# iyak/RNAelem

Hardware: AMD Instinct MI355X
Metric: train-iter seqs/sec (inside+outside) (higher is better)
Workload: dtype f64; 1 GPU; 10000 synthetic RNAs L=200, pattern ((.*.)), W=50 C=30 min_bpp=1e-4 T2004, x0 lambda=(1,1), one (fn,gr) eval per step; n_seq=10000, seq_len=200, pattern=((.*.)), bpp_filter=cached (computed once at load_batch, 0.1 s incl. plan), n_skipped=0

## Files before the change

### rnaelem_amd/api.py

```python
import ctypes as C
import json
import os

import numpy as np

HERE = os.path.dirname(os.path.abspath(__file__))
LIB_PATH = os.path.join(HERE, "libelemdp.so")

NO_RSS, NO_PROFILE, NO_ENERGY, THETA_SOFTMAX, LIK_RATIO = 1, 2, 4, 8, 16
DBG_FIX_RSS, DBG_NO_TURN = 1 << 9, 1 << 10

SYMBOLS = ["elemdp_last_error", "elemdp_abi_version", "elemdp_set_data_dir", "elemdp_create", "elemdp_destroy",
           "elemdp_n_param", "elemdp_n_state", "elemdp_n_node", "elemdp_initial_params", "elemdp_describe",
           "elemdp_set_option", "elemdp_load_batch", "elemdp_batch_bpp_eff", "elemdp_batch_pairs", "elemdp_useful_mask", "elemdp_useful_mask_host", "elemdp_live_blocks", "elemdp_live_blocks_host", "elemdp_live_blocks_inside", "elemdp_live_blocks_host_bits", "elemdp_train_eval",
           "elemdp_partial_len", "elemdp_train_partial", "elemdp_train_finish", "elemdp_set_finish_params", "elemdp_train_seq_stats", "elemdp_train_seq_counts",
           "elemdp_debug_tables", "elemdp_scan", "elemdp_pair_posteriors", "elemdp_pair_mea", "elemdp_sample", "elemdp_context_profile", "elemdp_node_profile", "elemdp_accessibility", "elemdp_node_mea", "elemdp_pair_conditional", "elemdp_pair_conditional_list", "elemdp_pair_list", "elemdp_last_timing", "elemdp_debug_profile", "elemdp_kernel_name", "elemdp_kmer_shuffle", "elemdp_epoch_permutation",
           "elemdp_comm_unique_id", "elemdp_comm_init", "elemdp_comm_destroy"]


class ModelDesc(C.Structure):
    _fields_ = [("pattern", C.c_char_p), ("energy_param", C.c_char_p), ("max_span", C.c_int32), ("max_iloop", C.c_int32),
                ("min_bpp", C.c_double), ("tau", C.c_double), ("flags", C.c_int32), ("device", C.c_int32)]


# ... 384 lines not shown
                r["structure_motif"] = sm.raw[lo:hi].decode("ascii")
                r["structure_none"] = sn.raw[lo:hi].decode("ascii")
            recs.append(r)
        return recs

    SAMPLED, NO_PARSE, REFUSED = 0, 1, 2

    def sample_structures(self, x, n_samples, seed=0, index_base=0):
        x = np.ascontiguousarray(x, dtype=np.float64)
        off = self._off
        n_samples = int(n_samples)
        nb = max(int(off[-1]) * max(n_samples, 0), 1)
        rss = C.create_string_buffer(nb)
        node = np.zeros(nb, dtype=np.uint8)
        logp = np.zeros(max(self.n_seq * max(n_samples, 0), 1))
        status = np.zeros(max(self.n_seq, 1), dtype=np.int32)
        self._check(self._lib.elemdp_sample(self._h, _dp(x), self.n_param, n_samples, int(seed) & (2 ** 64 - 1), int(index_base),
                                            rss, node.ctypes.data_as(C.POINTER(C.c_uint8)), _dp(logp), _i32(status)))
        raw = rss.raw.decode("ascii")
        out = []
        for k in range(self.n_seq):
            L, b = int(off[k + 1] - off[k]), int(off[k]) * n_samples
            out.append(([raw[b + t * L:b + (t + 1) * L] for t in range(n_samples)], node[b:b + n_samples * L].reshape(n_samples, L).copy(),
                        logp[k * n_samples:(k + 1) * n_samples].copy(), int(status[k])))
        return out

    CONTEXT_LETTERS = "OLRHBIM"

    def context_profiles(self, x):
        x = np.ascontiguousarray(x, dtype=np.float64)
        off = self._off
        n_pos = int(off[-1]) if off is not None else 0
        prof = np.zeros(max(7 * n_pos, 1))
        self._check(self._lib.elemdp_context_profile(self._h, _dp(x), self.n_param, _dp(prof)))
        return [prof[7 * int(off[k]):7 * int(off[k + 1])].reshape(-1, 7).copy() for k in range(self.n_seq)]

    def node_profiles(self, x):
        x = np.ascontiguousarray(x, dtype=np.float64)
        off = self._off
        M = self.n_node
        n_pos = int(off[-1]) if off is not None else 0
        prof = np.zeros(max(M * n_pos, 1))
        self._check(self._lib.elemdp_node_profile(self._h, _dp(x), self.n_param, _dp(prof)))
        return [prof[M * int(off[k]):M * int(off[k + 1])].reshape(-1, M).copy() for k in range(self.n_seq)]

    def accessibility(self, x, max_width=16):
        x = np.ascontiguousarray(x, dtype=np.float64)
        off = self._off
        U = int(max_width)
        n_pos = int(off[-1]) if off is not None else 0
        acc = np.zeros(max(max(U, 1) * n_pos, 1))
        self._check(self._lib.elemdp_accessibility(self._h, _dp(x), self.n_param, U, _dp(acc)))
        return [acc[U * int(off[k]):U * int(off[k + 1])].reshape(-1, U).copy() for k in range(self.n_seq)]

    def mea_alignments(self, x, gamma=1.0, max_sites=1, profile=False):
        x = np.ascontiguousarray(x, dtype=np.float64)
        off = self._off
        M, K, n = self.n_node, int(max_sites), max(self.n_seq, 0)
        n_pos = int(off[-1]) if off is not None else 0
        kk = min(max(K, 1), 64)
        prof = np.zeros(max(M * n_pos, 1)) if profile else None
        node = np.zeros(max(kk * n_pos, 1), dtype=np.uint8)
        ns = np.zeros(max(n, 1), dtype=np.int32)
        s0, s1 = np.zeros(max(n * kk, 1), dtype=np.int32), np.zeros(max(n * kk, 1), dtype=np.int32)
        sc, cf = np.zeros(max(n * kk, 1)), np.zeros(max(n * kk, 1))
        self._check(self._lib.elemdp_node_mea(self._h, _dp(x), self.n_param, float(gamma), K, _dp(prof), _u8(node), _i32(ns),
                                              _i32(s0), _i32(s1), _dp(sc), _dp(cf)))
        out = []
        for k in range(self.n_seq):
            a, b, m = int(off[k]), int(off[k + 1]), int(ns[k])
            L = b - a
            rec = dict(rows=node[K * a:K * a + m * L].reshape(m, L).copy(), start=s0[k * K:k * K + m].copy(),
                       end=s1[k * K:k * K + m].copy(), score=sc[k * K:k * K + m].copy(), confidence=cf[k * K:k * K + m].copy())
            if profile:
                rec["profile"] = prof[M * a:M * b].reshape(L, M).copy()
            out.append(rec)
        return out

    def last_timing(self):
        ms = np.zeros(3)
        self._lib.elemdp_last_timing(self._h, _dp(ms), 3)
        return ms

    def profile(self):
        c = np.zeros(16)
        self._lib.elemdp_debug_profile(self._h, _dp(c), 16)
        return c

    def kernel_name(self):
        return self._lib.elemdp_kernel_name().decode()


def alignment_confidence(profile, psihat):
    profile = np.asarray(profile, dtype=np.float64)
    psihat = np.asarray(psihat, dtype=np.int64)
    if profile.ndim != 2 or psihat.shape != (profile.shape[0],):
        raise ValueError("alignment_confidence: an (L, M) profile and L node indices are expected")
    if psihat.size and (psihat.min() < 0 or psihat.max() >= profile.shape[1]):
        raise ValueError("alignment_confidence: node index out of range")
    return profile[np.arange(profile.shape[0]), psihat]
```

### rnaelem_amd/csrc/engine.cpp

```cpp
#include <hip/hip_runtime_api.h>

#include <algorithm>
#include <chrono>
#include <cmath>
#include <cstdio>
#include <cstdlib>
#include <cstring>
#include <fstream>
#include <limits>
#include <memory>
#include <numeric>
#include <random>
#include <sstream>
#include <stdexcept>
#include <string>
#include <mutex>
#include <thread>
#include <vector>

#include <dlfcn.h>

#include "../../include/elemdp.h"
#include "access_rules.h"
#include "automaton.h"
// ... 105 lines not shown
  DevBuf d_plans, dmin, e_stack, e_ext, e_ml, e_close, e_hp, off_outer, off_inner, off_left, off_right, cursor, items,
      item_in, idx_inner, idx_left, idx_right, items_inner, items_left, items_right;
  DevBuf useful;
  bool useful_built = false;
  DevBuf blocks, blk_max;
  int64_t n_blocks = 0;
  int blk_cpb = 0, blk_cap = 0;
  std::vector<int32_t> h_blk_max, h_blk_grid;
  std::vector<int32_t> h_blk_grid_in;
  bool blk_all = false;
  bool blk_two = false;
  int64_t n_cells = 0;
  bool permuted = false;
  bool inner_only = false;
  bool sorted = true;
  PlanKernelArgs ka;
  int64_t n_items = 0;
  PlanArrays arrays() const {
    PlanArrays a;
    a.dmin = dmin.as<int16_t>();
    a.e_stack = e_stack.as<double>(); a.e_ext = e_ext.as<double>(); a.e_ml = e_ml.as<double>();
    a.e_close = e_close.as<double>(); a.e_hp = e_hp.as<double>();
    a.by_outer_off = off_outer.as<int32_t>(); a.by_inner_off = off_inner.as<int32_t>();
    a.by_left_off = off_left.as<int32_t>(); a.by_right_off = off_right.as<int32_t>();
    a.cursor = cursor.as<int32_t>();
    a.items = items.as<LoopItem>(); a.item_in = item_in.as<uint8_t>();
    a.by_inner_idx = idx_inner.as<int32_t>(); a.by_left_idx = idx_left.as<int32_t>(); a.by_right_idx = idx_right.as<int32_t>();
    a.items_inner = items_inner.as<LoopItem>(); a.items_left = items_left.as<LoopItem>(); a.items_right = items_right.as<LoopItem>();
    return a;
  }
};

}

class Engine {
 public:
  explicit Engine(const elemdp_model_desc& d);
  ~Engine();

  void useful_mask(int idx, uint8_t* mask, int cap);
  void live_blocks(int idx, int32_t* counts, void* records, int stride, int32_t* cpb_cap, int32_t* taken, bool inside = false);
  int n_param() const { return au_.n_theta() + 2; }
  int n_state() const { return au_.S(); }
  int n_node() const { return au_.M(); }
  const Automaton& automaton() const { return au_; }
  const AutomatonLayout& layout() const { return lays_.shadow >= 0 ? lays_ : lay_; }
  bool softmax() const { return flags_ & ELEMDP_THETA_SOFTMAX; }

  void load_batch(const uint8_t* seq, const int32_t* off, const uint8_t* qual, const int32_t* qoff, const char* fix, int n);
  void train_partial(const double* x, int n_param, void* partial, bool device_ptr, bool reduce = false);
  void train_finish(const double* reduced, double* fn, double* gr, double* sum_eff, int32_t* n_skipped);
  void scan(const double* x, int n_param, elemdp_scan_out* out);
  struct MeaOut { double gamma; char* structure; double* score; };
  void pair_posteriors(const double* x, int n_param, double min_prob, int64_t* n_pairs, double* unpaired, const MeaOut* mea = nullptr);
  void pair_list(int32_t* seq, int32_t* i, int32_t* j, double* p, int64_t cap);
  struct CondOut { double gamma; double* exist; double* unpaired[2]; char* structure[2]; double* shift; };
  void pair_conditional(const double* x, int n_param, double min_prob, int64_t* n_pairs, const CondOut& out);
  void cond_list(int32_t* seq, int32_t* i, int32_t* j, double* p_motif, double* p_none, int64_t cap);
  struct SampleOut { char* rss; uint8_t* node; double* logp; int32_t* status; };
  void sample_structures(const double* x, int n_param, int n_samples, uint64_t seed, int64_t index_base, const SampleOut& out);
  void context_profile(const double* x, int n_param, double* profile);
  void node_profile(const double* x, int n_param, double* profile);
  void accessibility(const double* x, int n_param, int max_width, double* access);
  struct NodeMeaOut { double* profile; uint8_t* node; int32_t* n_sites; int32_t* start; int32_t* end; double* score; double* conf; };
  void node_mea(const double* x, int n_param, double gamma, int max_sites, const NodeMeaOut& out);
  int partial_len() const { return 4 + 2 * au_.n_theta() + 4; }
  void set_option(const std::string& key, double v);
  void comm_init(int rank, int world, const void* id);
  void comm_destroy();
  bool has_comm() const { return comm_ != nullptr; }

  int n_seq() const { return n_seq_; }
  const std::vector<SeqPlan>& plans() const { return h_plans_; }
  void seq_stats(double* out, int n);
  void seq_counts(double* out, int n);
  bool bpp_eff_known() const {
    if (!streaming_) return true;
    for (char c : st_have_eff_) if (!c) return false;
    return true;
  }
  void debug_tables(double* inside, double* outside, double* inside_o, double* outside_o, double* ENo, double* ENx, double* EH);
  void batch_pairs(int idx, uint8_t* kept, double* lnbpp, int cap);
  double last_ms[3] = {0, 0, 0};

 private:
  void upload_params(const double* x, const AutomatonLayout& lay, bool trivial);
 public:
  void set_theta_from(const double* x);
 private:
  struct BatchShape {
    std::vector<SeqPlan> plans;
    int Lmax = 0, Wmax = 0, nword_max = 0;
    int64_t n_bases = 0, n_pos = 0, n_words = 0, n_cells = 0;
  };
  BatchShape check_batch(const uint8_t* seq, const int32_t* off, const uint8_t* qual, const int32_t* qoff, const char* fix, int n) const;
  void stage_batch(BatchShape&& b, const uint8_t* seq, const int32_t* off, const uint8_t* qual, const int32_t* qoff, const char* fix,
                   std::vector<uint8_t>& h_seq, std::vector<uint32_t>& fix_bits);
  const uint32_t* bpp_filter(const std::vector<uint32_t>& fix_bits);
  void bpp_chunks(bool lin);
  void bpp_lin_chunk(int first, int count, int64_t cells, double* lnbpp);
  void bpp_log_chunk(int first, int count, int64_t cells, double* lnbpp);
  void resident_plan(const uint32_t* mask);
  void build_planset(PlanSet& ps, int first, int count, const uint32_t* d_okbits);
  void ensure_sorted_plan();
  void ensure_useful_mask();
  bool ensure_live_blocks(int cpb, int cap, bool inside_too);
  bool loop_prepass_ok(bool sched1) const;
  bool loop_outside_ok(bool sched1) const;
  int live_span_for(int cpb) const;
  bool lists_wanted() const;
  LdsLayout lds_layout(const AutomatonLayout& lay, int Lmax, int nword_max, bool scan) const;
  DpArgs base_args(const AutomatonLayout& lay, const int32_t* d_ints, const double* d_params, const PlanSet& ps,
                   const uint32_t* d_okbits, int S);
  SlotRequest slot_request(int S, int row, bool scan, int n_want, int group = 0, int pair_row = 0) const;
  void run_train();
  void run_train_batch();
  void run_lin_batch();
  int prepare_lin(LinArgs& a, bool sched1, bool dense_too = false, int n_eval = 0, int group_cap = 8192);
  template <class Work> void sweep_groups(const LinArgs& a, int n, const int32_t* h_ord, const int32_t* d_ord, const SeqPlan* d_sorted,
                                          int gsz, int ns, Work work);
  struct ScanPos {
    DevBuf start, inner, end, ys, ye, exist;
    ScanPos(size_t n_seqpos, int n) {
      start.alloc(8 * n_seqpos); inner.alloc(8 * n_seqpos); end.alloc(8 * (n_seqpos + n));
      ys.alloc(4 * (size_t)n); ye.alloc(4 * (size_t)n); exist.alloc(8 * (size_t)n);
    }
  };
  int prepare_scan(LinArgs& a, const ScanPos& pos);
  int read_flagged(std::vector<int32_t>* list = nullptr);
  DpArgs log_scan_args(bool sums_on_batch, int* n_blocks);
  int log_chunk(bool sums_on_batch, int n_blocks, int n_log) const;
  PairArgs pair_batch_args() const;
  void pair_plane_fields(PairArgs& pa, const LinArgs& a) const;
  void require_resident(const char* what, int n_param_in);
  template <class Fill, class Group> int scan_sums(const ScanPos& pos, Fill fill, Group group, std::vector<int32_t>* flagged = nullptr);
  template <class Fill, class Behind> void scan_log_form(bool sums_on_batch, int n_flagged, Fill fill, Behind behind);
  int node_profile_device(const char* what, const double* x, int n_param_in);
  TrArgs log_pipeline_args();
  void init_device();
  void flatten_automaton();
  void poison_tables();
  void lin_weights(int first = 0, int count = 0);
  void upload_automaton();
  bool opt_prune_ = true;
  int opt_eval_first_ = 0, opt_eval_count_ = 0;
  std::vector<int32_t> h_order_r_;
  DevBuf d_order_r_, d_plans_sorted_r_;
  int range_key_[2] = {-1, -1};
  bool opt_det_ = false;
  bool opt_fast_ = true;
  bool opt_poison_ = false;
  void require_device() const;
  bool has_device_ = false;
  int want_device_ = -1;
  Rccl::Comm comm_ = nullptr;
  int comm_rank_ = 0, comm_world_ = 1;
  bool streaming_ = false;
  int st_chunk_ = 0, opt_max_resident_ = 0;
  bool inner_ = false;
  size_t slot_budget_ = 0, st_slot_budget_ = 0;
  std::vector<uint8_t> st_seq_, st_qual_;
  std::vector<char> st_fix_;
  std::vector<double> st_rows_;
  std::unique_ptr<Engine> sub_[2];
  std::vector<std::pair<std::string, double>> opt_log_;
  elemdp_model_desc desc_;
  std::string desc_pattern_, desc_par_;
  bool desc_has_par_ = false;
  bool should_stream(const BatchShape& b);
  void stream_setup(const uint8_t* seq, const int32_t* off, const uint8_t* qual, const int32_t* qoff, const char* fix,
                    BatchShape&& b);
  void stream_load_chunk(int k, Engine& e);
  std::vector<std::vector<uint32_t>> st_mask_;
  std::vector<std::vector<double>> st_eff_;
  std::vector<char> st_have_eff_;
  const uint32_t* preset_bits_ = nullptr;
  const double* preset_eff_ = nullptr;
  size_t preset_words_ = 0;
  size_t bits_words_ = 0;
  void set_filter_preset(const uint32_t* bits, size_t words, const double* eff) { preset_bits_ = bits; preset_words_ = words; preset_eff_ = eff; }
  void filter_result(std::vector<uint32_t>& bits, std::vector<double>& eff) {
    bits.resize(bits_words_);
    HIP_OK(hipMemcpyAsync(bits.data(), d_okbits1_.as<void>(), sizeof(uint32_t) * bits_words_, hipMemcpyDeviceToHost, st_));
    HIP_OK(hipStreamSynchronize(st_));
    eff.resize(h_plans_.size());
    for (size_t k = 0; k < h_plans_.size(); ++k) eff[k] = h_plans_[k].bpp_eff;
  }
  void stream_subs();
  template <class Checked, class Work> void stream_call(int n_param_in, Checked checked, Work work);
  void stream_train(const double* x, int n_param, void* partial, bool device_ptr, bool reduce);
  void stream_scan(const double* x, int n_param, elemdp_scan_out* out);
  void stream_pairs(const double* x, int n_param, double min_prob, double* unpaired, const MeaOut* mea);
  void stream_samples(const double* x, int n_param, int n_samples, uint64_t seed, int64_t index_base, const SampleOut& out);
  void stream_cond(const double* x, int n_param, double min_prob, const CondOut& out);
  DevBuf d_pr_kept_, d_pr_koff_, d_pr_cnt_, d_pr_off_, d_pr_P_, d_pr_unp_, d_pr_si_, d_pr_sj_, d_pr_sp_;
  DevBuf d_pl_seq_, d_pl_i_, d_pl_j_, d_pl_p_;
  int64_t n_pairs_ = -1;
  DevBuf d_mea_M_, d_mea_ch_, d_mea_s_, d_mea_sc_;
  DevBuf d_sm_rss_, d_sm_node_, d_sm_logp_, d_sm_status_, d_sm_stack_;
  DevBuf d_cd_kept_, d_cd_koff_, d_cd_cnt_, d_cd_off_, d_cd_P_, d_cd_z_, d_cd_unp_[2], d_cd_exist_, d_cd_shift_, d_cd_si_, d_cd_sj_, d_cd_sp_[2];
  DevBuf d_cl_seq_, d_cl_i_, d_cl_j_, d_cl_p_[2];
  int64_t n_cond_ = -1;
  DevBuf d_cd_M_, d_cd_ch_, d_cd_s_[2], d_cd_sc_;
  DevBuf d_cx_cells_, d_cx_o_, d_cx_prof_;
  DevBuf d_ac_T_, d_ac_vec_, d_ac_out_;
  DevBuf d_nd_lists_, d_nd_prof_;
  DevBuf d_nm_lists_, d_nm_bp_, d_nm_node_, d_nm_ns_, d_nm_s0_, d_nm_s1_, d_nm_sc_, d_nm_cf_;

  Automaton au_;
  EnergyTables et_;
  AutomatonLayout lay_, lay0_, layr_;
  std::vector<int32_t> ints_, ints0_, intsr_;
  bool linear_ok_ = true;
  int flags_, max_span_, max_iloop_;
  bool loops_finite_ = false;
  double min_bpp_, tau_;
  int m_min() const { return (flags_ & ELEMDP_DBG_NO_TURN) ? 4 : 10; }
  int min_span() const { return (flags_ & ELEMDP_DBG_NO_TURN) ? 1 : 5; }
  int device_ = -1, n_cu_ = 256;
  hipStream_t st_ = nullptr;
  hipEvent_t ev_[4] = {nullptr, nullptr, nullptr, nullptr};
  static constexpr int kMaxGroupStreams = 4;
  hipStream_t gs_[kMaxGroupStreams] = {nullptr, nullptr, nullptr, nullptr};
  void need_group_streams(int ns) {
    for (int k = 1; k < ns && k < kMaxGroupStreams; ++k)
      if (!gs_[k]) HIP_OK(hipStreamCreateWithFlags(&gs_[k], hipStreamNonBlocking));
  }
  hipEvent_t gdone_[kMaxGroupStreams] = {}, gstart_ = nullptr;
  int opt_group_streams_ = 2;
  int group_streams(bool concurrent) const {
    return (concurrent && opt_group_streams_ >= 2) ? std::min(opt_group_streams_, kMaxGroupStreams) : 1;
  }
  DevBuf d_et_, d_xet_, d_ints_, d_ints0_, d_params_, d_params0_, d_counter_, d_lay_, d_lay0_, d_layr_, d_intsr_;
// ... 132 lines not shown
    HIP_OK(hipMemcpy(d_xet_.as<void>(), x.get(), sizeof(EnergyTables), hipMemcpyHostToDevice));
    std::unique_ptr<BppCandTable> ct(new BppCandTable);
    build_bpp_cand(*x, ct.get());
    bpp_.cand.alloc(sizeof(BppCandTable));
    HIP_OK(hipMemcpy(bpp_.cand.as<void>(), ct.get(), sizeof(BppCandTable), hipMemcpyHostToDevice));
  }
  d_ints0_.upload(ints0_, st_);
  upload_automaton();
  d_lay0_.alloc(sizeof(AutomatonLayout));
  d_lin_.alloc(sizeof(double) * (kLinEth + au_.n_theta() + 1));
  HIP_OK(hipMemcpyAsync(d_lay0_.as<void>(), &lay0_, sizeof(AutomatonLayout), hipMemcpyHostToDevice, st_));
  d_params_.alloc(sizeof(ParamBlock) + sizeof(double) * (au_.n_theta() + 1));
  d_params0_.alloc(sizeof(ParamBlock) + sizeof(double));
  d_counter_.alloc(sizeof(int32_t));
  d_partial_.alloc(sizeof(double) * partial_len());
  {
    ParamBlock pb;
    pb.lambda[0] = pb.lambda[1] = 1.;
    pb.log_tau = 0.;
    pb.lam_same = 1;
    pb.pad = 0;
    HIP_OK(hipMemcpyAsync(d_params0_.as<void>(), &pb, sizeof(pb), hipMemcpyHostToDevice, st_));
  }
  HIP_OK(hipStreamSynchronize(st_));
}

void Engine::comm_init(int rank, int world, const void* id) {
  require_device();
  if (!id || world < 1 || rank < 0 || rank >= world) throw ArgError("elemdp_comm_init: bad rank / world / id");
  Rccl& r = Rccl::get();
  if (!r.ok()) throw HipError("no HIP device available for the collective: librccl.so could not be loaded");
  DeviceGuard dg(device_);
  comm_destroy();
  Rccl::UniqueId uid;
  std::memcpy(&uid, id, sizeof(uid));
  RCCL_OK(r.CommInitRank(&comm_, world, uid, rank));
  comm_rank_ = rank;
  comm_world_ = world;
}

void Engine::comm_destroy() {
  if (comm_) { DeviceGuard dg(device_); (void)Rccl::get().CommDestroy(comm_); comm_ = nullptr; comm_world_ = 1; comm_rank_ = 0; }
}

Engine::~Engine() {
  if (!has_device_) return;
  DeviceGuard dg(device_);
  comm_destroy();
  if (st_) (void)hipStreamSynchronize(st_);
  for (auto& e : ev_) if (e) (void)hipEventDestroy(e);
  for (int k = 0; k < kMaxGroupStreams; ++k) {
    if (gdone_[k]) (void)hipEventDestroy(gdone_[k]);
    if (k && gs_[k]) (void)hipStreamDestroy(gs_[k]);
  }
  if (gstart_) (void)hipEventDestroy(gstart_);
  if (st_) (void)hipStreamDestroy(st_);
}

void Engine::set_option(const std::string& key, double v) {
  if (key == "max_resident") { opt_max_resident_ = (int)v; return; }
  if (key == "slots") opt_slots_ = (int)v;
  else if (key == "keep_lnbpp") opt_keep_lnbpp_ = v != 0;
  else if (key == "first_pass_only") opt_first_pass_only_ = v != 0;
  else if (key == "profile") opt_profile_ = v != 0;
  else if (key == "two_streams") {}
  else if (key == "group_streams") opt_group_streams_ = (int)v;
  else if (key == "pipeline") {
    if ((int)v != 3 && (int)v != 4) throw ArgError("option pipeline: 4 (scaled linear, default) or 3 (log space); the fused kernel (2) is retired");
    opt_pipeline_ = (int)v;
  }
  else if (key == "group") opt_group_ = (int)v;
  else if (key == "node_rules") {
    if (v < 1 || v > NR_ALL) throw ArgError("node_rules: 1 .. 63 (bits: L <- L, rule 3a, rule 5a, left base of rules 1a / 1b, rule 8, right base of rules 1a / 1b)");
    opt_node_rules_ = (int)v;
  }
  else if (key == "access_terms") {
    if (v < 1 || v > 15) throw ArgError("access_terms: 1 .. 15 (bits: loop runs, exterior, tails behind a branch, leading bases of a multi-loop)");
    opt_access_terms_ = (int)v;
  }
  else if (key == "schedule") opt_schedule_ = (int)v;
  else if (key == "dbg") opt_dbg_ = (int)v;
  else if (key == "bpp_log") opt_bpp_log_ = v != 0;
  else if (key == "poison") opt_poison_ = v != 0;
  else if (key == "fast") opt_fast_ = v != 0;
  else if (key == "deterministic") opt_det_ = v != 0;
  else if (key == "sorted_plan") opt_sorted_plan_ = v != 0;
  else if (key == "useful_mask") opt_useful_mask_ = v != 0;
  else if (key == "live_blocks") {
    if (v < 0 || v > 2) throw ArgError("live_blocks: 0, 1 or 2");
    opt_live_blocks_ = (int)v;
  }
  else if (key == "loop_prepass") opt_loop_prepass_ = v != 0;
  else if (key == "loop_outside") opt_loop_outside_ = v != 0;
  else if (key == "live_span") {
    if (v < 0 || v > lin_live_span_max()) throw ArgError("live_span: 0 (default) or cells per block .. " + std::to_string(lin_live_span_max()));
    opt_live_span_ = (int)v;
  }
  else if (key == "useful_mask_lds_kb") {
    if (v < 0 || v > 150) throw ArgError("useful_mask_lds_kb: 0 .. 150");
    opt_useful_lds_kb_ = (int)v;
  }
  else if (key == "eval_first") opt_eval_first_ = (int)v;
  else if (key == "eval_count") opt_eval_count_ = (int)v;
  else if (key == "prune") {
    opt_prune_ = v != 0;
    slots_.invalidate();
    flatten_automaton();
    if (has_device_) { DeviceGuard dg(device_); HIP_OK(hipStreamSynchronize(st_)); upload_automaton(); }
  }
  else throw ArgError("unknown option: " + key);
  for (auto& m : st_mask_) m.clear();
  opt_log_.emplace_back(key, v);
  for (auto& e : sub_) if (e) e->set_option(key, v);
}

void Engine::set_theta_from(const double* x) {
  const int nt = au_.n_theta();
  theta_.assign(x, x + nt);
  if (softmax()) {
    for (int r = 0; r < au_.n_rows(); ++r) {
      const int o = au_.row_offset(r), w = au_.row_width(r);
      double tot = -std::numeric_limits<double>::infinity();
      for (int c = 0; c < w; ++c) {
        const double a = tot, b = x[o + c];
        tot = (b == -INFINITY) ? a : (a == -INFINITY) ? b : (a < b ? b + std::log1p(std::exp(a - b)) : a + std::log1p(std::exp(b - a)));
      }
      for (int c = 0; c < w; ++c) theta_[o + c] = x[o + c] - tot;
    }
  }
}

void Engine::upload_params(const double* x, const AutomatonLayout& lay, bool) {
  const int nt = au_.n_theta();
  set_theta_from(x);
  std::vector<double> blob(sizeof(ParamBlock) / sizeof(double) + nt + 1, 0.);
  ParamBlock pb;
  pb.lambda[0] = x[nt];
  pb.lambda[1] = x[nt + 1];
  pb.log_tau = std::log(tau_);
  pb.lam_same = (x[nt] == x[nt + 1]) ? 1 : 0;
  pb.pad = 0;
  std::memcpy(blob.data(), &pb, sizeof(pb));
  std::copy(theta_.begin(), theta_.end(), blob.begin() + sizeof(ParamBlock) / sizeof(double));
  HIP_OK(hipMemcpyAsync(d_params_.as<void>(), blob.data(), blob.size() * sizeof(double), hipMemcpyHostToDevice, st_));
  make_lin_params(lay_, ints_.data(), theta_.data(), tau_, (flags_ & ELEMDP_NO_PROFILE) != 0, &h_lin_);
  d_lin_.alloc(sizeof(double) * (h_lin_.size() + 1));
  HIP_OK(hipMemcpyAsync(d_lin_.as<void>(), h_lin_.data(), h_lin_.size() * sizeof(double), hipMemcpyHostToDevice, st_));
  make_lin_params(lays_, intss_.data(), theta_.data(), tau_, (flags_ & ELEMDP_NO_PROFILE) != 0, &h_lins_);
  d_lins_.alloc(sizeof(double) * (h_lins_.size() + 1));
  HIP_OK(hipMemcpyAsync(d_lins_.as<void>(), h_lins_.data(), h_lins_.size() * sizeof(double), hipMemcpyHostToDevice, st_));
  HIP_OK(hipStreamSynchronize(st_));
  (void)lay;
}

LdsLayout Engine::lds_layout(const AutomatonLayout& lay, int Lmax, int nword_max, bool scan) const {
  LdsLayout l;
  int o = 0;
  auto take = [&](int bytes) { int p = o; o += (bytes + 15) & ~15; return p; };
  l.theta = take(8 * (lay.n_theta + 1));
  l.en_o = take(8 * (lay.n_theta + 1));
  l.en_x = take(8 * (lay.n_theta + 1));
  l.eh = take(8 * 4);
  l.zs = take(8 * 8);
  l.ws = take(8 * (Lmax + 1));
  l.post = take(scan ? 8 * 3 * (Lmax + 1) : 16);
  l.ints = take(4 * lay.n_small);
// ... 16 lines not shown
  t0 = t1;
}

void Engine::build_planset(PlanSet& ps, int first, int count, const uint32_t* d_okbits) {
  ps.first = first;
  ps.count = count;
  ps.h.assign(h_plans_.begin() + first, h_plans_.begin() + first + count);
  int64_t dmin_b = 0, cell_b = 0, off_b = 0, bits_end = 0, ncell_max = 0, blk_b = 0;
  int lmax = 0, wmax1 = 0;
  for (auto& p : ps.h) {
    const int64_t nc = (int64_t)(p.L + 1) * (p.W + 1);
    p.dmin_base = dmin_b; p.cell_base = cell_b; p.off_base = off_b; p.item_base = 0; p.n_items = 0;
    p.blk_base = blk_b >= 0 ? (int32_t)blk_b : 0;
    if (blk_b >= 0) { blk_b += live_blocks_records(p.L, p.W); if (blk_b > 0x7fffffffll) blk_b = -1; }
    dmin_b += p.L + 1; cell_b += nc; off_b += nc + 1;
    bits_end = std::max<int64_t>(bits_end, p.bits_base + (nc + 31) / 32);
    ncell_max = std::max(ncell_max, nc);
    lmax = std::max(lmax, (int)p.L);
    wmax1 = std::max(wmax1, (int)p.W + 1);
  }
  ps.n_cells = cell_b;
  ps.n_blocks = blk_b;
  ps.useful_built = false;
  ps.blk_cpb = ps.blk_cap = 0;
  d_okbits_end_.alloc(sizeof(uint32_t) * (size_t)bits_end);
  ps.d_plans.upload(ps.h, st_);
  const bool chunked = ps.inner_only;
  ps.dmin.alloc(sizeof(int16_t) * dmin_b, chunked);
  for (DevBuf* b : {&ps.e_stack, &ps.e_ext, &ps.e_ml, &ps.e_close, &ps.e_hp}) b->alloc(sizeof(double) * cell_b, chunked);
  for (DevBuf* b : {&ps.off_outer, &ps.off_inner, &ps.off_left, &ps.off_right, &ps.cursor}) b->alloc(sizeof(int32_t) * off_b, chunked);
  d_nitems_.alloc(sizeof(int32_t) * count);
  PlanKernelArgs a;
  a.et = d_et_.as<EnergyTables>();
  a.b.seq = d_seq_.as<uint8_t>(); a.b.ws = d_ws_.as<double>(); a.b.unp = d_unp_.as<uint8_t>();
  a.b.ndot = (flags_ & ELEMDP_DBG_FIX_RSS) ? d_ndot_.as<int32_t>() : nullptr;
  a.okbits = d_okbits;
  a.okbits_end = d_okbits_end_.as<uint32_t>();
  a.ncell_max = (int32_t)ncell_max;
  a.n_roles = ps.inner_only ? 1 : 3;
  a.lmax = lmax;
  a.wmax1 = wmax1;
  a.nword_max = (int32_t)((ncell_max + 31) / 32);
  a.plans = ps.d_plans.as<SeqPlan>();
  a.first = 0; a.count = count;
  a.p = ps.arrays();
  a.no_ene = (flags_ & ELEMDP_NO_ENERGY) ? 1 : 0;
  a.min_span = min_span();
  a.fix_rss = (flags_ & ELEMDP_DBG_FIX_RSS) ? 1 : 0;
  a.count_fast = (loops_finite_ && !a.fix_rss && !getenv("ELEMDP_PLAN_ENUM_COUNT")) ? 1 : 0;
  HIP_OK(launch_plan_cells(a, d_nitems_.as<int32_t>(), st_));
  std::vector<int32_t> n_items(count);
  HIP_OK(hipMemcpyAsync(n_items.data(), d_nitems_.as<void>(), sizeof(int32_t) * count, hipMemcpyDeviceToHost, st_));
  HIP_OK(hipStreamSynchronize(st_));
  int64_t ib = 0;
  for (int k = 0; k < count; ++k) {
    ps.h[k].n_items = n_items[k]; ps.h[k].item_base = ib; ib += n_items[k];
    a.nitems_max = std::max(a.nitems_max, n_items[k]);
  }
  ps.n_items = ib;
  if (getenv("ELEMDP_PLAN_DEBUG")) fprintf(stderr, "planset: %d sequences, %lld items, largest %d, cells %lld\n", count, (long long)ib, a.nitems_max, (long long)ncell_max);
  ps.d_plans.upload(ps.h, st_);
  ps.items.alloc(sizeof(LoopItem) * ib, true);
  ps.item_in.alloc(ib, true);
  for (DevBuf* b : {&ps.idx_inner, &ps.idx_left, &ps.idx_right}) b->alloc(sizeof(int32_t) * ib, true);
  if (ps.permuted) for (DevBuf* b : {&ps.items_inner, &ps.items_left, &ps.items_right}) b->alloc(sizeof(LoopItem) * (ib + 1), true);
  a.plans = ps.d_plans.as<SeqPlan>();
  a.p = ps.arrays();
  a.sort_roles = (ps.inner_only || opt_det_ || opt_pipeline_ != 4 || opt_sorted_plan_) ? 1 : 0;
  HIP_OK(launch_plan_items(a, st_));
  if (ps.permuted && !plan_copies_fused(a)) HIP_OK(launch_permute_items(a, st_));
  HIP_OK(hipStreamSynchronize(st_));
  ps.sorted = a.sort_roles != 0;
  ps.ka = a;
}

void Engine::ensure_useful_mask() {
  if (plan_.useful_built || plan_.count <= 0) return;
  plan_.useful.alloc((size_t)plan_.n_cells);
  plan_.ka.p.useful = plan_.useful.as<uint8_t>();
  plan_.ka.m_min = m_min();
  HIP_OK(launch_useful_mask(plan_.ka, (size_t)plan_.n_cells, (size_t)opt_useful_lds_kb_ * 1024, st_));
  plan_.useful_built = true;
  plan_.blk_cpb = plan_.blk_cap = 0;
}

bool Engine::ensure_live_blocks(int cpb, int cap, bool inside_too) {
  if (plan_.count <= 0 || plan_.n_blocks <= 0 || cpb < kLiveCpbMin || cap < cpb || cap > kLiveSpanMax) return false;
  ensure_useful_mask();
  if (plan_.blk_cpb == cpb && plan_.blk_cap == cap && plan_.blk_all == (opt_live_blocks_ >= 2) && (plan_.blk_two || !inside_too)) return true;
  plan_.blocks.alloc(sizeof(LiveBlock) * (inside_too ? 2 : 1) * (size_t)plan_.n_blocks);
  plan_.blk_max.alloc(sizeof(int32_t) * 6 * (size_t)plan_.ka.wmax1);
  PlanKernelArgs a = plan_.ka;
  a.p.useful = plan_.useful.as<uint8_t>();
  a.p.blocks = plan_.blocks.as<LiveBlock>();
  a.p.blocks_in = inside_too ? a.p.blocks + (size_t)plan_.n_blocks : nullptr;
  a.blk_max = plan_.blk_max.as<int32_t>();
  a.live_cpb = cpb; a.live_cap = cap;
  HIP_OK(launch_live_blocks(a, (size_t)plan_.n_blocks, st_));
  plan_.h_blk_max.assign(6 * (size_t)a.wmax1, 0);
  HIP_OK(hipMemcpyAsync(plan_.h_blk_max.data(), a.blk_max, sizeof(int32_t) * 6 * (size_t)a.wmax1, hipMemcpyDeviceToHost, st_));
  HIP_OK(hipStreamSynchronize(st_));
  plan_.h_blk_grid.assign((size_t)a.wmax1, 0);
  plan_.h_blk_grid_in.assign((size_t)a.wmax1, 0);
  for (int d = 0; d < a.wmax1; ++d) {
    const int32_t* mi = plan_.h_blk_max.data() + 3 * (size_t)a.wmax1;
    const long long nb = plan_.h_blk_max[a.wmax1 + d], nw = plan_.h_blk_max[2 * a.wmax1 + d];
    const long long nbi = mi[a.wmax1 + d], nwi = mi[2 * a.wmax1 + d];
    plan_.h_blk_grid[d] = (opt_live_blocks_ >= 2 || nb * 100 <= nw * kLiveKeepPct) ? plan_.h_blk_max[d] : -1;
    plan_.h_blk_grid_in[d] = (opt_live_blocks_ >= 2 || nbi * 100 <= nwi * kLiveKeepPct) ? mi[d] : -1;
    if (getenv("ELEMDP_PLAN_DEBUG"))
      fprintf(stderr, "live blocks d %d: most %d, blocks %lld, working without lists %lld%s; inside behind the loop pre-pass: most %d, blocks %lld, working without lists %lld%s\n",
              d, plan_.h_blk_max[d], nb, nw, plan_.h_blk_grid[d] < 0 ? " (consecutive)" : "", mi[d], nbi, nwi, plan_.h_blk_grid_in[d] < 0 ? " (consecutive)" : "");
  }
  plan_.blk_all = opt_live_blocks_ >= 2;
  plan_.blk_two = inside_too;
  plan_.blk_cpb = cpb; plan_.blk_cap = cap;
  return true;
}

void Engine::ensure_sorted_plan() {
  if (plan_.sorted || plan_.count <= 0) return;
  HIP_OK(launch_plan_sort(plan_.ka, st_));
  if (plan_.permuted) HIP_OK(launch_permute_items(plan_.ka, st_));
  HIP_OK(hipStreamSynchronize(st_));
  plan_.sorted = true;
}

SlotRequest Engine::slot_request(int S, int row, bool scan, int n_want, int group, int pair_row) const {
  SlotRequest r;
  r.S = S; r.row = row; r.scan = scan; r.n_want = n_want; r.group = group; r.pair_row = pair_row;
  r.opt_slots = opt_slots_; r.n_cu = n_cu_;
  r.Lmax = Lmax_; r.Wmax = Wmax_; r.S_dense = au_.S();
  r.budget = slot_budget_;
  return r;
}

DpArgs Engine::base_args(const AutomatonLayout& lay, const int32_t* d_ints, const double* d_params, const PlanSet& ps,
                         const uint32_t* d_okbits, int S) {
  DpArgs a;
  std::memset(&a, 0, sizeof(a));
  a.lay = lay;
  a.layp = (&lay == &lay0_) ? d_lay0_.as<AutomatonLayout>() : d_lay_.as<AutomatonLayout>();
  a.ints = d_ints;
  a.params = d_params;
  a.no_prf = (flags_ & ELEMDP_NO_PROFILE) ? 1 : 0;
  a.m_min = m_min();
  a.no_rss = (flags_ & ELEMDP_NO_RSS) ? 1 : 0;
  a.plans = ps.d_plans.as<SeqPlan>();
  a.n_seq = ps.count;
  a.counter = d_counter_.as<int32_t>();
  a.b.seq = d_seq_.as<uint8_t>(); a.b.ws = d_ws_.as<double>(); a.b.unp = d_unp_.as<uint8_t>();
  a.b.ndot = nullptr;
  a.okbits = d_okbits;
  a.p = ps.arrays();
  a.band_in = slots_.band_in.as<double>(); a.band_out = slots_.band_out.as<double>();
  a.ext_in = slots_.ext_in.as<double>(); a.ext_out = slots_.ext_out.as<double>();
  a.band_stride = (size_t)kNumBandStates * (Wmax_ + 1) * (Lmax_ + 1) * S;
  a.ext_stride = (size_t)(Lmax_ + 1) * S;
  a.tmp = slots_.tmp.as<double>();
  a.tmp_stride = a.ext_stride;
  return a;
}

void Engine::load_batch(const uint8_t* seq, const int32_t* off, const uint8_t* qual, const int32_t* qoff, const char* fix,
                        int n) {
  require_device();
  DeviceGuard dg(device_);
  n_seq_ = 0;
  n_pairs_ = -1;
  n_cond_ = -1;
  streaming_ = false;
  train_rows_ = false;
  BatchShape shape = check_batch(seq, off, qual, qoff, fix, n);
  h_seq_off_.assign(off, off + n + 1);
  h_qual_off_.assign(qoff, qoff + n + 1);
  if (should_stream(shape)) { stream_setup(seq, off, qual, qoff, fix, std::move(shape)); return; }
  std::vector<uint8_t> h_seq;
  std::vector<uint32_t> fix_bits;
  stage_batch(std::move(shape), seq, off, qual, qoff, fix, h_seq, fix_bits);
  const bool rss = !(flags_ & ELEMDP_DBG_FIX_RSS) && !(flags_ & ELEMDP_NO_RSS);
  d_ncanon_.alloc(sizeof(int32_t) * n);
  d_plans_all_.upload(h_plans_, st_);
  BatchArrays b;
  b.seq = d_seq_.as<uint8_t>(); b.ws = d_ws_.as<double>(); b.unp = d_unp_.as<uint8_t>(); b.ndot = nullptr;
  HIP_OK(launch_mask(b, d_plans_all_.as<SeqPlan>(), n, min_span(), rss, d_okbits0_.as<uint32_t>(), d_ncanon_.as<int32_t>(), st_));
  std::vector<int32_t> ncanon(n);
  HIP_OK(hipMemcpyAsync(ncanon.data(), d_ncanon_.as<void>(), sizeof(int32_t) * n, hipMemcpyDeviceToHost, st_));
  HIP_OK(hipStreamSynchronize(st_));
  for (int k = 0; k < n; ++k) h_plans_[k].n_canonical = ncanon[k];
  dbg_lap("load: uploads + canonical mask");
  resident_plan(bpp_filter(fix_bits));
  h_seq_.swap(h_seq);
  n_seq_ = n;
  opt_eval_first_ = opt_eval_count_ = 0;
  range_key_[0] = range_key_[1] = -1;
}

Engine::BatchShape Engine::check_batch(const uint8_t* seq, const int32_t* off, const uint8_t* qual, const int32_t* qoff,
                                       const char* fix, int n) const {
  if (n <= 0 || !seq || !off || !qual || !qoff) throw ArgError("load_batch: empty batch or null pointer");
  if ((flags_ & ELEMDP_DBG_FIX_RSS) && !fix) throw ArgError("load_batch: ELEMDP_DBG_FIX_RSS needs fix_rss strings");
  BatchShape b;
  b.plans.assign(n, SeqPlan());
  for (int k = 0; k < n; ++k) {
    const int L = off[k + 1] - off[k];
    if (L <= 0) throw ArgError("load_batch: empty sequence");
    if (L > 32000) throw ArgError("load_batch: sequence longer than 32000");
    if (qoff[k + 1] - qoff[k] != L + 1) throw ArgError("bad seq format. (quality must have L+1 entries)");
// ... 186 lines not shown
    HIP_OK(hipMemcpyAsync(h, a.prof, sizeof(h), hipMemcpyDeviceToHost, st_));
    HIP_OK(hipStreamSynchronize(st_));
    static const char* nm[8] = {"stage", "stems", "loops generic", "loops 1xn / bulge", "special shapes", "barrier 1", "unary", "barrier 2"};
    for (int dir = 0; dir < 2; ++dir) {
      unsigned long long tot = 0;
      for (int k = 0; k < 8; ++k) tot += h[dir * 8 + k];
      for (int k = 0; k < 8; ++k)
        fprintf(stderr, "[elemdp bpp prof] %s %-18s %6.2f %%  %.3g cycles per sequence\n", dir ? "out" : "in ", nm[k],
                tot ? 100. * (double)h[dir * 8 + k] / (double)tot : 0., (double)h[dir * 8 + k] / count);
    }
  }
}

void Engine::bpp_log_chunk(int first, int count, int64_t cells, double* lnbpp) {
  BppScratch& f = bpp_;
  PlanSet& tmp = f.plan;
  tmp.inner_only = true;
  build_planset(tmp, first, count, d_okbits0_.as<uint32_t>());
  dbg_lap("load: plan of the unfiltered mask (chunk)");
  const size_t band1 = (size_t)kNumBandStates * (Wmax_ + 1) * (Lmax_ + 1), ext1 = (size_t)(Lmax_ + 1);
  f.planes_finite = false;
  for (DevBuf* b : {&f.band_in, &f.band_out}) b->alloc(band1 * count * sizeof(double), true);
  for (DevBuf* b : {&f.ext_in, &f.ext_out}) b->alloc(ext1 * count * sizeof(double), true);
  f.tmp.alloc(ext1 * 3 * count * sizeof(double), true);
  const SeqPlan& last = h_plans_.back();
  if (f.zero_ws.alloc(sizeof(double) * (size_t)(last.pos_base + last.L + 1)))
    HIP_OK(hipMemsetAsync(f.zero_ws.as<void>(), 0, f.zero_ws.bytes(), st_));
  std::vector<int32_t> order(count);
  std::iota(order.begin(), order.end(), 0);
  std::stable_sort(order.begin(), order.end(), [&](int a2, int b2) { return tmp.h[a2].L > tmp.h[b2].L; });
  f.order.upload(order, st_);
  const int stride = 10;
  f.rows.alloc(sizeof(double) * stride * count);
  TrArgs a;
  std::memset(&a, 0, sizeof(a));
  a.lay = lay0_;
  a.layp = d_lay0_.as<AutomatonLayout>();
  a.ints = d_ints0_.as<int32_t>();
  a.layp_r = a.layp; a.ints_r = a.ints;
  a.params = d_params0_.as<double>();
  a.no_prf = 1;
  a.m_min = m_min();
  a.plans = tmp.d_plans.as<SeqPlan>();
  a.grp = f.order.as<int32_t>();
  a.b.seq = d_seq_.as<uint8_t>(); a.b.ws = f.zero_ws.as<double>(); a.b.unp = d_unp_.as<uint8_t>(); a.b.ndot = nullptr;
  a.okbits = d_okbits0_.as<uint32_t>();
  a.p = tmp.arrays();
  a.band_in = f.band_in.as<double>(); a.band_out = f.band_out.as<double>();
  a.ext_in = f.ext_in.as<double>(); a.ext_out = f.ext_out.as<double>();
  a.band_stride = band1; a.ext_stride = ext1;
  a.tmp = f.tmp.as<double>(); a.tmp_stride = ext1;
  a.seq_out = f.rows.as<double>(); a.out_stride = stride;
  BppOut o;
  o.okbits_out = d_okbits1_.as<uint32_t>();
  o.kept = f.kept.as<int32_t>();
  o.log_min_bpp = std::log(min_bpp_);
  o.lnbpp = lnbpp;
  HIP_OK(hipMemsetAsync(f.rows.as<void>(), 0, sizeof(double) * stride * count, st_));
  const int Lg = tmp.h[order[0]].L;
  HIP_OK(launch_bpp_group(a, o, count, Lg, std::min(Lg, max_span_), st_));
}

void Engine::resident_plan(const uint32_t* mask) {
  const int n = (int)h_plans_.size();
  if (mask != d_okbits1_.as<uint32_t>())
    HIP_OK(hipMemcpyAsync(d_okbits1_.as<void>(), mask, sizeof(uint32_t) * bits_words_, hipMemcpyDeviceToDevice, st_));
  plan_.permuted = true;
  build_planset(plan_, 0, n, d_okbits1_.as<uint32_t>());
  dbg_lap("load: plan of the filtered mask");
  for (int k = 0; k < n; ++k) { plan_.h[k].bpp_eff = h_plans_[k].bpp_eff; plan_.h[k].n_canonical = h_plans_[k].n_canonical; }
  plan_.d_plans.upload(plan_.h, st_);
  h_plans_ = plan_.h;
  d_order_.upload(h_order_, st_);
  std::vector<SeqPlan> sorted(n);
  for (int k = 0; k < n; ++k) { sorted[k] = h_plans_[h_order_[k]]; sorted[k].index = h_order_[k]; }
  d_plans_sorted_.upload(sorted, st_);
  HIP_OK(hipStreamSynchronize(st_));
  d_xwc_.alloc(sizeof(double) * 10 * (size_t)n_cells_total_);
  d_flagged_.alloc(sizeof(int32_t) * ((size_t)n + 1));
  out_stride_ = 6 + 2 * au_.n_theta() + 4;
  d_seq_out_.alloc(sizeof(double) * (size_t)out_stride_ * n);
  HIP_OK(hipMemsetAsync(d_seq_out_.as<void>(), 0, sizeof(double) * (size_t)out_stride_ * n, st_));
  slots_.invalidate();
  HIP_OK(hipStreamSynchronize(st_));
  dbg_lap("load: weights / output buffers");
}

bool Engine::should_stream(const BatchShape& b) {
  if (inner_) return false;
  if (opt_max_resident_ > 0) return (int)b.plans.size() > opt_max_resident_;
  size_t free_b = 0, total_b = 0;
  if (hipMemGetInfo(&free_b, &total_b) != hipSuccess) return false;
  const size_t held = slots_.held_bytes(TableSlots::Held::Stream) + d_xwc_.bytes() + d_xwi_.bytes();
  return (double)b.n_cells * 600.0 > 0.5 * (double)(free_b + held);
}

void Engine::stream_setup(const uint8_t* seq, const int32_t* off, const uint8_t* qual, const int32_t* qoff, const char* fix,
                          BatchShape&& b) {
  const int n = (int)b.plans.size();
  h_plans_ = std::move(b.plans);
  st_seq_.assign(seq + off[0], seq + off[n]);
  st_qual_.assign(qual + qoff[0], qual + qoff[n]);
  if (fix) st_fix_.assign(fix + off[0], fix + off[n]); else st_fix_.clear();
  st_slot_budget_ = 0;
  if (opt_max_resident_ > 0) st_chunk_ = opt_max_resident_;
  else {
    size_t free_b = 0, total_b = 0;
    HIP_OK(hipMemGetInfo(&free_b, &total_b));
    const double per_seq = (double)b.n_cells / n * 600.0;
    st_chunk_ = (int)std::max(256.0, std::min((double)n, 0.2 * (double)free_b / per_seq));
    st_slot_budget_ = (size_t)(0.2 * (double)free_b);
  }
  st_rows_.clear();
  {
    const int nchunks = (n + st_chunk_ - 1) / st_chunk_;
    st_mask_.assign(nchunks, {});
    st_eff_.assign(nchunks, {});
    st_have_eff_.assign(nchunks, 0);
  }
  slots_.release();
  d_xwc_.reset(); d_xwi_.reset();
  streaming_ = true;
  n_seq_ = n;
}

void Engine::stream_subs() {
  for (auto& e : sub_) {
    if (e) { e->slot_budget_ = st_slot_budget_; continue; }
    elemdp_model_desc d = desc_;
    d.pattern = desc_pattern_.c_str();
    d.energy_param = desc_has_par_ ? desc_par_.c_str() : nullptr;
    d.device = device_;
    e.reset(new Engine(d));
    e->inner_ = true;
    e->slot_budget_ = st_slot_budget_;
    for (auto const& kv : opt_log_) e->set_option(kv.first, kv.second);
  }
}

void Engine::stream_load_chunk(int k, Engine& e) {
  const int c0 = k * st_chunk_, c1 = std::min(n_seq_, c0 + st_chunk_);
  std::vector<int32_t> off(c1 - c0 + 1), qoff(c1 - c0 + 1);
  for (int t = c0; t <= c1; ++t) { off[t - c0] = h_seq_off_[t] - h_seq_off_[c0]; qoff[t - c0] = h_qual_off_[t] - h_qual_off_[c0]; }
  const size_t s0 = (size_t)(h_seq_off_[c0] - h_seq_off_[0]), q0 = (size_t)(h_qual_off_[c0] - h_qual_off_[0]);
  const bool cached = k < (int)st_mask_.size() && !st_mask_[k].empty();
  if (cached) e.set_filter_preset(st_mask_[k].data(), st_mask_[k].size(), st_eff_[k].data());
  e.load_batch(st_seq_.data() + s0, off.data(), st_qual_.data() + q0, qoff.data(), st_fix_.empty() ? nullptr : st_fix_.data() + s0, c1 - c0);
  if (!cached && k < (int)st_mask_.size() && st_fix_.empty() && !(flags_ & ELEMDP_NO_RSS) && min_bpp_ > 0) e.filter_result(st_mask_[k], st_eff_[k]);
  for (int t = c0; t < c1; ++t) h_plans_[t].bpp_eff = e.h_plans_[t - c0].bpp_eff;
  if (k < (int)st_have_eff_.size()) st_have_eff_[k] = 1;
}

template <class Checked, class Work> void Engine::stream_call(int n_param_in, Checked checked, Work work) {
  if (n_param_in != n_param()) throw ArgError("n_param mismatch");
  checked();
  last_ms[0] = last_ms[1] = last_ms[2] = 0.;
  stream_subs();
  const int nchunks = (n_seq_ + st_chunk_ - 1) / st_chunk_;
  stream_load_chunk(0, *sub_[0]);
  for (int k = 0; k < nchunks; ++k) {
    Engine& cur = *sub_[k & 1];
    std::exception_ptr err;
    std::thread th;
    if (k + 1 < nchunks)
      th = std::thread([&, k] {
        try { stream_load_chunk(k + 1, *sub_[(k + 1) & 1]); } catch (...) { err = std::current_exception(); }
// ... 25 lines not shown
    for (int t = c0; t < c1; ++t) h_plans_[t].bpp_eff = e.plans()[t - c0].bpp_eff;
  });
  if (comm_ && reduce) {
    HIP_OK(hipMemcpyAsync(d_partial_.as<void>(), total.data(), sizeof(double) * np, hipMemcpyHostToDevice, st_));
    RCCL_OK(Rccl::get().AllReduce(d_partial_.as<void>(), d_partial_.as<void>(), (size_t)np, Rccl::kDouble, Rccl::kSum, comm_, st_));
    HIP_OK(hipMemcpyAsync(total.data(), d_partial_.as<void>(), sizeof(double) * np, hipMemcpyDeviceToHost, st_));
    HIP_OK(hipStreamSynchronize(st_));
  }
  if (device_ptr) HIP_OK(hipMemcpy(partial, total.data(), sizeof(double) * np, hipMemcpyHostToDevice));
  else std::memcpy(partial, total.data(), sizeof(double) * np);
}

void Engine::stream_scan(const double* x, int n_param_in, elemdp_scan_out* out) {
  const int nt = au_.n_theta();
  std::vector<double> en(nt, 0.), en_k(nt);
  stream_call(n_param_in, [&] { if (!out) throw ArgError("scan: null output"); }, [&](int c0, int, Engine& e) {
    const size_t so = (size_t)(h_seq_off_[c0] - h_seq_off_[0]), qo = (size_t)(h_qual_off_[c0] - h_qual_off_[0]);
    elemdp_scan_out o = *out;
    if (o.start) o.start += so;
    if (o.inner) o.inner += so;
    if (o.end) o.end += qo;
    if (o.psihat) o.psihat += so;
    if (o.rss) o.rss += so;
    if (o.ys) o.ys += c0;
    if (o.ye) o.ye += c0;
    if (o.exist_prob) o.exist_prob += c0;
    o.en = out->en ? en_k.data() : nullptr;
    e.scan(x, n_param_in, &o);
    if (out->en) for (int t = 0; t < nt; ++t) en[t] += en_k[t];
  });
  if (out->en) std::copy(en.begin(), en.end(), out->en);
}

TrArgs Engine::log_pipeline_args() {
  const int S = au_.S();
  TrArgs a;
  std::memset(&a, 0, sizeof(a));
  a.lay = lay_;
  a.layp = d_lay_.as<AutomatonLayout>();
  a.ints = d_ints_.as<int32_t>();
  a.params = d_params_.as<double>();
  a.no_prf = (flags_ & ELEMDP_NO_PROFILE) ? 1 : 0;
  a.m_min = m_min();
  a.no_rss = (flags_ & ELEMDP_NO_RSS) ? 1 : 0;
  a.first_pass_only = opt_first_pass_only_ ? 1 : 0;
  a.lik_ratio = (flags_ & ELEMDP_LIK_RATIO) ? 1 : 0;
  a.schedule = (opt_schedule_ == 1 && linear_ok_ && !opt_first_pass_only_) ? 1 : 0;
  a.layp_r = d_layr_.as<AutomatonLayout>();
  a.ints_r = d_intsr_.as<int32_t>();
  a.plans = plan_.d_plans.as<SeqPlan>();
  a.b.seq = d_seq_.as<uint8_t>(); a.b.ws = d_ws_.as<double>(); a.b.unp = d_unp_.as<uint8_t>(); a.b.ndot = nullptr;
  a.okbits = d_okbits1_.as<uint32_t>();
  a.p = plan_.arrays();
  a.band_in = slots_.band_in.as<double>(); a.band_out = slots_.band_out.as<double>();
  a.ext_in = slots_.ext_in.as<double>(); a.ext_out = slots_.ext_out.as<double>();
  a.band_stride = (size_t)kNumBandStates * (Wmax_ + 1) * (Lmax_ + 1) * S;
  a.ext_stride = (size_t)(Lmax_ + 1) * S;
  a.tmp = slots_.tmp.as<double>();
  a.tmp_stride = a.ext_stride;
  a.seq_out = d_seq_out_.as<double>();
  a.out_stride = out_stride_;
  return a;
}

void Engine::run_train_batch() {
  if (opt_eval_count_ > 0 && !(opt_eval_first_ == 0 && opt_eval_count_ == n_seq_))
    throw ArgError("eval_first / eval_count: the log-space pipeline (pipeline 3) evaluates the whole batch");
  slots_.ensure(slot_request(au_.S(), 0, false, n_seq_, opt_group_ > 0 ? opt_group_ : 4096), free_device_bytes());
  TrArgs a = log_pipeline_args();
  slots_.set_holds(TableSlots::Holds::DenseLog);
  const int n_slots = slots_.n();
  HIP_OK(hipMemsetAsync(d_seq_out_.as<void>(), 0, sizeof(double) * (size_t)out_stride_ * n_seq_, st_));
  HIP_OK(hipEventRecord(ev_[1], st_));
  for (int g0 = 0; g0 < n_seq_; g0 += n_slots) {
    const int G = std::min(n_slots, n_seq_ - g0);
    a.grp = d_order_.as<int32_t>() + g0;
    const int Lg = h_plans_[h_order_[g0]].L;
    HIP_OK(launch_train_group(a, G, Lg, std::min(Lg, max_span_), st_));
  }
  HIP_OK(hipEventRecord(ev_[2], st_));
  HIP_OK(launch_reduce(d_seq_out_.as<double>(), out_stride_, n_seq_, au_.n_theta(), d_partial_.as<double>(), st_));
}

void Engine::poison_tables() {
  if (!opt_poison_) return;
  for (DevBuf* b : {&slots_.band_in, &slots_.band_out, &slots_.a_in, &slots_.a_out})
    if (b->bytes()) HIP_OK(hipMemsetAsync(b->as<void>(), 0xff, b->bytes(), st_));
}

void Engine::lin_weights(int first, int count) {
  LinWeightArgs w;
  const PlanArrays pa = plan_.arrays();
  w.e_stack = pa.e_stack; w.e_ext = pa.e_ext; w.e_ml = pa.e_ml; w.e_close = pa.e_close; w.e_hp = pa.e_hp;
  w.items = pa.items;
  w.items_inner = pa.items_inner; w.items_left = pa.items_left; w.items_right = pa.items_right;
  w.n_cells = (size_t)n_cells_total_; w.n_items = (size_t)plan_.n_items;
  if (count > 0 && count < n_seq_) {
    const SeqPlan& p0 = h_plans_[first];
    const SeqPlan& p1 = h_plans_[first + count - 1];
    w.cell_first = (size_t)p0.cell_base;
    w.cell_count = (size_t)(p1.cell_base + (int64_t)(p1.L + 1) * (p1.W + 1) - p0.cell_base);
  }
  w.params = d_params_.as<double>();
  w.xwc = d_xwc_.as<double>(); w.xwi = nullptr;
  HIP_OK(launch_lin_weights(w, st_));
}

int Engine::prepare_lin(LinArgs& a, bool sched1, bool dense_too, int n_eval, int group_cap) {
  const bool shadow = sched1 && lays_.shadow >= 0;
  const AutomatonLayout& L = shadow ? lays_ : lay_;
  const int S = L.S, Sa = std::max(lay_.S, lays_.S), nap = std::max(lay_.ap_rs, lays_.ap_rs);
  const int row = std::max(std::max(lay_.tab_row, lays_.tab_row), dense_too ? kNumBandStates * lay_.S : 0);
  const int n_need = n_eval > 0 ? std::min(n_eval, n_seq_) : n_seq_;
  const size_t free_b = free_device_bytes();
  const int group = balanced_group(lin_group_bytes(Lmax_, Wmax_, row, Sa, nap), n_need, group_cap, opt_group_, slot_budget_, free_b,
                                   slots_.held_bytes(TableSlots::Held::Group));
  slots_.ensure(slot_request(Sa, row, false, n_need, group, nap), free_b);
  const int gsz = even_groups(n_need, slots_.n());
  std::memset(&a, 0, sizeof(a));
  a.lay = L;
  a.layp = shadow ? d_lays_.as<AutomatonLayout>() : d_lay_.as<AutomatonLayout>();
  a.ints = shadow ? d_intss_.as<int32_t>() : d_ints_.as<int32_t>();
  a.params = d_params_.as<double>();
  a.lin = shadow ? d_lins_.as<double>() : d_lin_.as<double>();
  a.fast = (opt_fast_ && !(flags_ & ELEMDP_DBG_FIX_RSS)) ? 1 : 0;
  a.no_prf = (flags_ & ELEMDP_NO_PROFILE) ? 1 : 0;
  a.m_min = m_min();
  a.no_rss = (flags_ & ELEMDP_NO_RSS) ? 1 : 0;
  a.lik_ratio = (flags_ & ELEMDP_LIK_RATIO) ? 1 : 0;
  a.ext_block = (flags_ & (ELEMDP_DBG_NO_TURN | ELEMDP_DBG_FIX_RSS)) ? 1 : 4;
  a.plans = plan_.d_plans.as<SeqPlan>();
  a.b.seq = d_seq_.as<uint8_t>(); a.b.ws = d_ws_.as<double>(); a.b.unp = d_unp_.as<uint8_t>(); a.b.ndot = nullptr;
  a.ews = d_ews_.as<double>();
  a.okbits = d_okbits1_.as<uint32_t>();
  a.p = plan_.arrays();
  a.xwc = d_xwc_.as<double>(); a.xwc_stride = (size_t)n_cells_total_;
  a.xwi = nullptr; a.xwi_stride = 0;
  a.band_in = slots_.band_in.as<double>(); a.band_out = slots_.band_out.as<double>();
  a.ext_in = slots_.ext_in.as<double>(); a.ext_out = slots_.ext_out.as<double>();
  a.band_stride = slots_.band_stride();
  a.ext_stride = (size_t)(Lmax_ + 1) * S;
  a.zs = slots_.zs.as<double>();
  a.a_in = slots_.a_in.as<double>(); a.a_out = slots_.a_out.as<double>();
  a.a_stride = (size_t)(Wmax_ + 1) * (Lmax_ + 1) * L.ap_rs;
  a.okbits_end = d_okbits_end_.as<uint32_t>();
  a.lmax = Lmax_;
  a.nword_max = nword_max_;
  a.seq_out = d_seq_out_.as<double>();
  a.out_stride = out_stride_;
  a.schedule = sched1 ? 1 : 0;
  a.flagged = d_flagged_.as<int32_t>();
  a.dbg = opt_dbg_;
  a.prof = nullptr;
  if (opt_profile_) {
    d_prof_.alloc(sizeof(long long) * 16 * 64);
    HIP_OK(hipMemsetAsync(d_prof_.as<void>(), 0, sizeof(long long) * 16 * 64, st_));
    a.prof = d_prof_.as<long long>();
  }
  a.n_stage = (L.n_ints <= 4096 && !(opt_dbg_ & 8)) ? L.n_ints : L.n_small;
  return gsz;
}

template <class Work>
void Engine::sweep_groups(const LinArgs& a, int n, const int32_t* h_ord, const int32_t* d_ord, const SeqPlan* d_sorted, int gsz,
                          int ns, Work work) {
  const int slots_each = slots_.n() / ns;
  if (ns > 1) {
    int n_groups = (n + slots_each - 1) / slots_each;
    n_groups = ((n_groups + ns - 1) / ns) * ns;
    gsz = (n + n_groups - 1) / n_groups;
  }
  need_group_streams(ns);
  if (ns > 1) {
    HIP_OK(hipEventRecord(gstart_, st_));
    for (int k = 1; k < ns; ++k) HIP_OK(hipStreamWaitEvent(gs_[k], gstart_, 0));
  }
  int gi = 0;
  for (int g0 = 0; g0 < n; g0 += gsz, ++gi) {
    const int k = gi % ns;
    const size_t k0 = (size_t)k * slots_each;
    LinArgs ak = a;
    ak.band_in += k0 * a.band_stride; ak.band_out += k0 * a.band_stride;
    ak.ext_in += k0 * a.ext_stride; ak.ext_out += k0 * a.ext_stride;
    ak.zs += 4 * k0;
    ak.a_in += k0 * a.a_stride; ak.a_out += k0 * a.a_stride;
    if (a.tr_ext) ak.tr_ext += k0 * a.ext_stride;
    if (a.trace_stack) ak.trace_stack += k0 * a.trace_stack_stride;
    ak.grp = d_ord + g0;
    ak.plans_slot = d_sorted + g0;
    const int Lg = h_plans_[h_ord[g0]].L;
    work(ak, k0, std::min(gsz, n - g0), Lg, std::min(Lg, max_span_), gs_[k]);
  }
  for (int k = 1; k < ns; ++k) {
    HIP_OK(hipEventRecord(gdone_[k], gs_[k]));
    HIP_OK(hipStreamWaitEvent(st_, gdone_[k], 0));
  }
}

int Engine::read_flagged(std::vector<int32_t>* list) {
  int32_t n_flagged = 0;
  HIP_OK(hipMemcpyAsync(&n_flagged, d_flagged_.as<void>(), sizeof(int32_t), hipMemcpyDeviceToHost, st_));
  HIP_OK(hipStreamSynchronize(st_));
  if (list) {
    list->resize(n_flagged);
    if (n_flagged) HIP_OK(hipMemcpy(list->data(), d_flagged_.as<int32_t>() + 1, sizeof(int32_t) * n_flagged, hipMemcpyDeviceToHost));
  }
  n_flagged_last_ = n_flagged;
  return n_flagged;
}

void Engine::run_lin_batch() {
  const bool sched1 = opt_schedule_ == 1 && linear_ok_ && !opt_first_pass_only_ && lay_.s00 == 0 && lays_.shadow >= 0;
  LinArgs a;
  const bool ranged = opt_eval_count_ > 0 && !(opt_eval_first_ == 0 && opt_eval_count_ == n_seq_);
  const int r0 = ranged ? opt_eval_first_ : 0, n_ev = ranged ? opt_eval_count_ : n_seq_;
  if (r0 < 0 || n_ev <= 0 || r0 + n_ev > n_seq_) throw ArgError("eval_first / eval_count outside the resident batch");
  int gsz = prepare_lin(a, sched1, false, n_ev);
  if (opt_useful_mask_) ensure_useful_mask();
  a.p.useful = opt_useful_mask_ ? plan_.useful.as<uint8_t>() : nullptr;
  a.loop_pre = (opt_loop_prepass_ && opt_useful_mask_ && loop_prepass_ok(sched1)) ? 1 : 0;
  a.loop_post = (opt_loop_outside_ && opt_useful_mask_ && !opt_det_ && loop_prepass_ok(sched1) && loop_outside_ok(sched1)) ? 1 : 0;
  a.in_d0 = first_inside_diagonal(min_span(), m_min());
  if (lists_wanted()) {
    const int cpb = lin_train_cpb(a), cap = live_span_for(cpb);
    if (cpb > 0 && ensure_live_blocks(cpb, cap, a.loop_pre != 0 || a.loop_post != 0)) {
      a.p.blocks = plan_.blocks.as<LiveBlock>();
      a.p.blocks_in = plan_.blk_two ? a.p.blocks + (size_t)plan_.n_blocks : nullptr;
      a.live_span = cap;
      a.blk_grid = plan_.h_blk_grid.data();
      a.blk_grid_in = plan_.h_blk_grid_in.data();
    }
  }
  const int32_t* h_ord = h_order_.data();
  const int32_t* d_ord = d_order_.as<int32_t>();
  const SeqPlan* d_sorted = d_plans_sorted_.as<SeqPlan>();
  if (ranged) {
    if (range_key_[0] != r0 || range_key_[1] != n_ev || (int)h_order_r_.size() != n_ev) {
      h_order_r_.clear();
      for (int idx : h_order_) if (idx >= r0 && idx < r0 + n_ev) h_order_r_.push_back(idx);
      std::vector<SeqPlan> sorted(n_ev);
      for (int k = 0; k < n_ev; ++k) { sorted[k] = h_plans_[h_order_r_[k]]; sorted[k].index = h_order_r_[k]; }
      HIP_OK(hipStreamSynchronize(st_));
      d_order_r_.upload(h_order_r_, st_);
      d_plans_sorted_r_.upload(sorted, st_);
      HIP_OK(hipStreamSynchronize(st_));
      range_key_[0] = r0; range_key_[1] = n_ev;
    }
    h_ord = h_order_r_.data();
    d_ord = d_order_r_.as<int32_t>();
    d_sorted = d_plans_sorted_r_.as<SeqPlan>();
    gsz = even_groups(n_ev, slots_.n());
  }
  HIP_OK(hipMemsetAsync(d_seq_out_.as<double>() + (size_t)r0 * out_stride_, 0, sizeof(double) * (size_t)out_stride_ * n_ev, st_));
  HIP_OK(hipMemsetAsync(d_flagged_.as<void>(), 0, sizeof(int32_t), st_));
  if (opt_det_) {
    a.det = 1;
    a.det_nslot = (Lmax_ + 1 + std::max(1, kThreads / a.lay.S) - 1) / std::max(1, kThreads / a.lay.S) + 1;
    const size_t bytes = sizeof(double) * (size_t)n_seq_ * a.det_nslot * out_stride_;
    d_det_.alloc(bytes);
    HIP_OK(hipMemsetAsync(d_det_.as<void>(), 0, bytes, st_));
    a.det_rows = d_det_.as<double>();
  }
  HIP_OK(hipEventRecord(ev_[1], st_));
  lin_weights(r0, n_ev);
  poison_tables();
  const int ns = group_streams(n_ev >= 64 && slots_.n() >= 64 && !opt_profile_);
  sweep_groups(a, n_ev, h_ord, d_ord, d_sorted, gsz, ns, [&](const LinArgs& ak, size_t, int G, int Lg, int Wg, hipStream_t st) {
    HIP_OK(launch_lin_group(ak, G, Lg, Wg, opt_first_pass_only_, st));
  });
  const int n_flagged = read_flagged();
  if (opt_profile_) {
    std::vector<long long> hp(16 * 64);
    HIP_OK(hipMemcpy(hp.data(), d_prof_.as<void>(), sizeof(long long) * 16 * 64, hipMemcpyDeviceToHost));
    last_prof.assign(16, 0);
    for (size_t k = 0; k < hp.size(); ++k) last_prof[k % 16] += hp[k];
  }
  if (n_flagged == 0) slots_.set_holds(TableSlots::Holds::Linear, a.lay.S);
  else slots_.set_holds(TableSlots::Holds::DenseLog);
  if (n_flagged > 0) {
    ensure_sorted_plan();
    TrArgs t = log_pipeline_args();
    const int n_dense = (int)std::max<size_t>(1, std::min<size_t>((size_t)slots_.n(), (slots_.band_stride() * (size_t)slots_.n()) / t.band_stride));
    for (int g0 = 0; g0 < n_flagged; g0 += n_dense) {
      const int G = std::min(n_dense, n_flagged - g0);
      t.grp = d_flagged_.as<int32_t>() + 1 + g0;
      HIP_OK(launch_train_group(t, G, Lmax_, Wmax_, st_));
    }
  }
  HIP_OK(hipEventRecord(ev_[2], st_));
  HIP_OK(launch_reduce(d_seq_out_.as<double>() + (size_t)r0 * out_stride_, out_stride_, n_ev, au_.n_theta(), d_partial_.as<double>(), st_));
}

void Engine::run_train() {
  if (opt_pipeline_ == 3 || opt_det_) ensure_sorted_plan();
  if (opt_pipeline_ == 3) { run_train_batch(); return; }
  run_lin_batch();
}

void Engine::train_partial(const double* x, int n_param_in, void* partial, bool device_ptr, bool reduce) {
  require_device();
  DeviceGuard dg(device_);
  if (streaming_) { stream_train(x, n_param_in, partial, device_ptr, reduce); return; }
  if (n_seq_ <= 0 && !(comm_ && reduce)) throw StateError("train_eval before load_batch");
  if (n_param_in != n_param()) throw ArgError("n_param mismatch");
  HIP_OK(hipEventRecord(ev_[0], st_));
  last_x_.assign(x, x + n_param_in);
  upload_params(x, lay_, false);
  if (n_seq_ > 0) {
    train_rows_ = false;
    run_train();
    train_rows_ = true;
  } else {
    HIP_OK(hipMemsetAsync(d_partial_.as<void>(), 0, sizeof(double) * partial_len(), st_));
    HIP_OK(hipEventRecord(ev_[1], st_));
    HIP_OK(hipEventRecord(ev_[2], st_));
  }
  if (comm_ && reduce)
    RCCL_OK(Rccl::get().AllReduce(d_partial_.as<void>(), d_partial_.as<void>(), (size_t)partial_len(), Rccl::kDouble, Rccl::kSum, comm_, st_));
  HIP_OK(hipMemcpyAsync(partial, d_partial_.as<void>(), sizeof(double) * partial_len(),
                        device_ptr ? hipMemcpyDeviceToDevice : hipMemcpyDeviceToHost, st_));
  HIP_OK(hipEventRecord(ev_[3], st_));
  HIP_OK(hipStreamSynchronize(st_));
  float ms_all = 0, ms_k = 0;
  HIP_OK(hipEventElapsedTime(&ms_all, ev_[0], ev_[3]));
  HIP_OK(hipEventElapsedTime(&ms_k, ev_[1], ev_[2]));
  last_ms[0] = ms_all;
  last_ms[1] = ms_k;
  last_ms[2] = (opt_pipeline_ == 4) ? (double)n_flagged_last_ : 0.;
}

void Engine::train_finish(const double* r, double* fn, double* gr, double* sum_eff, int32_t* n_skipped) {
  const int nt = au_.n_theta();
  if (fn) *fn = r[0];
  if (sum_eff) *sum_eff = r[1];
  if (n_skipped) *n_skipped = (int32_t)std::llround(r[3]);
  if (!gr) return;
  const double* ENo = r + 4;
  const double* ENx = r + 4 + nt;
  const double* EHo = r + 4 + 2 * nt;
  const double* EHx = EHo + 2;
  int k = 0;
  if (softmax()) {
    if ((int)theta_.size() != nt) throw StateError("train_finish before any evaluation");
    for (int row = 0; row < au_.n_rows(); ++row) {
      const int o = au_.row_offset(row), w = au_.row_width(row);
      double tot = 0.;
      for (int c = 0; c < w; ++c) tot += ENo[o + c] - ENx[o + c];
      for (int c = 0; c < w; ++c) {
        const double tmp = ENo[o + c] - ENx[o + c];
        const double p = std::exp(theta_[o + c]);
        gr[k++] = (1 - p) * tmp - p * (tot - tmp);
      }
    }
  } else {
    for (int t = 0; t < nt; ++t) gr[k++] = ENo[t] - ENx[t];
  }
  gr[k++] = EHo[0] - EHx[0];
  gr[k++] = EHo[1] - EHx[1];
}

void Engine::seq_stats(double* out, int n) {
// ... 1319 lines not shown
int elemdp_debug_tables(elemdp_handle* h, double* inside, double* outside, double* inside_o, double* outside_o,
                        double* ENo, double* ENx, double* EH) {
  ELEMDP_TRY
  if (!h) throw elemdp::ArgError("null handle");
  h->e->debug_tables(inside, outside, inside_o, outside_o, ENo, ENx, EH);
  ELEMDP_CATCH
}
int elemdp_scan(elemdp_handle* h, const double* x, int32_t n_param, elemdp_scan_out* out) {
  ELEMDP_TRY
  if (!h || !x) throw elemdp::ArgError("elemdp_scan: null argument");
  h->e->scan(x, n_param, out);
  ELEMDP_CATCH
}
int elemdp_pair_posteriors(elemdp_handle* h, const double* x, int32_t n_param, double min_prob, int64_t* n_pairs, double* unpaired) {
  ELEMDP_TRY
  if (!h || !x || !n_pairs) throw elemdp::ArgError("elemdp_pair_posteriors: null argument");
  h->e->pair_posteriors(x, n_param, min_prob, n_pairs, unpaired);
  ELEMDP_CATCH
}
int elemdp_pair_mea(elemdp_handle* h, const double* x, int32_t n_param, double min_prob, double gamma, int64_t* n_pairs,
                    double* unpaired, char* structure, double* score) {
  ELEMDP_TRY
  if (!h || !x || !n_pairs) throw elemdp::ArgError("elemdp_pair_mea: null argument");
  const elemdp::Engine::MeaOut mea{gamma, structure, score};
  h->e->pair_posteriors(x, n_param, min_prob, n_pairs, unpaired, &mea);
  ELEMDP_CATCH
}
int elemdp_sample(elemdp_handle* h, const double* x, int32_t n_param, int32_t n_samples, uint64_t seed, int64_t index_base,
                  char* rss, uint8_t* node, double* logp, int32_t* status) {
  ELEMDP_TRY
  if (!h || !x) throw elemdp::ArgError("elemdp_sample: null argument");
  h->e->sample_structures(x, n_param, n_samples, seed, index_base, elemdp::Engine::SampleOut{rss, node, logp, status});
  ELEMDP_CATCH
}
int elemdp_context_profile(elemdp_handle* h, const double* x, int32_t n_param, double* profile) {
  ELEMDP_TRY
  if (!h || !x || !profile) throw elemdp::ArgError("elemdp_context_profile: null argument");
  h->e->context_profile(x, n_param, profile);
  ELEMDP_CATCH
}
int elemdp_accessibility(elemdp_handle* h, const double* x, int32_t n_param, int32_t max_width, double* access) {
  ELEMDP_TRY
  if (!h || !x || !access) throw elemdp::ArgError("elemdp_accessibility: null argument");
  h->e->accessibility(x, n_param, max_width, access);
  ELEMDP_CATCH
}
int elemdp_node_profile(elemdp_handle* h, const double* x, int32_t n_param, double* profile) {
  ELEMDP_TRY
  if (!h || !x || !profile) throw elemdp::ArgError("elemdp_node_profile: null argument");
  h->e->node_profile(x, n_param, profile);
  ELEMDP_CATCH
}
int elemdp_node_mea(elemdp_handle* h, const double* x, int32_t n_param, double gamma, int32_t max_sites, double* profile,
                    uint8_t* node, int32_t* n_sites, int32_t* site_start, int32_t* site_end, double* site_score, double* site_conf) {
  ELEMDP_TRY
  if (!h || !x) throw elemdp::ArgError("elemdp_node_mea: null argument");
  h->e->node_mea(x, n_param, gamma, max_sites, elemdp::Engine::NodeMeaOut{profile, node, n_sites, site_start, site_end, site_score, site_conf});
  ELEMDP_CATCH
}
int elemdp_pair_conditional(elemdp_handle* h, const double* x, int32_t n_param, double min_prob, double gamma, int64_t* n_pairs,
                            double* exist_prob, double* unpaired_motif, double* unpaired_none, char* structure_motif,
                            char* structure_none, double* shift) {
  ELEMDP_TRY
  if (!h || !x || !n_pairs) throw elemdp::ArgError("elemdp_pair_conditional: null argument");
  const elemdp::Engine::CondOut out{gamma, exist_prob, {unpaired_motif, unpaired_none}, {structure_motif, structure_none}, shift};
  h->e->pair_conditional(x, n_param, min_prob, n_pairs, out);
  ELEMDP_CATCH
}
int elemdp_pair_conditional_list(elemdp_handle* h, int32_t* seq, int32_t* i, int32_t* j, double* p_motif, double* p_none, int64_t cap) {
  ELEMDP_TRY
  if (!h) throw elemdp::ArgError("elemdp_pair_conditional_list: null handle");
  h->e->cond_list(seq, i, j, p_motif, p_none, cap);
  ELEMDP_CATCH
}
int elemdp_pair_list(elemdp_handle* h, int32_t* seq, int32_t* i, int32_t* j, double* p, int64_t cap) {
  ELEMDP_TRY
  if (!h) throw elemdp::ArgError("elemdp_pair_list: null handle");
  h->e->pair_list(seq, i, j, p, cap);
  ELEMDP_CATCH
}
int elemdp_last_timing(elemdp_handle* h, double* ms, int32_t n) {
  if (!h || !ms) return ELEMDP_EINVAL;
  for (int k = 0; k < n && k < 3; ++k) ms[k] = h->e->last_ms[k];
  return ELEMDP_OK;
}
int elemdp_debug_profile(elemdp_handle* h, double* cycles, int32_t n) {
  if (!h || !cycles) return ELEMDP_EINVAL;
  for (int k = 0; k < n && k < 16; ++k) cycles[k] = k < (int)h->e->last_prof.size() ? (double)h->e->last_prof[k] : 0.;
  return ELEMDP_OK;
}
int elemdp_kmer_shuffle(const uint8_t* codes, int32_t L, int32_t k, int32_t iter_cnt, uint8_t* out) {
  if (!codes || !out || L <= 0) return ELEMDP_EINVAL;
  int cnt = 0;
  for (int i = 0; i < L; ++i) cnt += codes[i] == codes[0];
  std::srand((unsigned)(cnt + iter_cnt));
  elemdp::kmer_shuffle(codes, L, k, out);
  return ELEMDP_OK;
}
int elemdp_epoch_permutation(int32_t n, int32_t seed, int32_t* perm) {
  if (n < 0 || (n > 0 && !perm)) return ELEMDP_EINVAL;
  std::vector<int32_t> v(n);
  std::iota(v.begin(), v.end(), 0);
  std::mt19937 m;
  m.seed((unsigned)seed);
  std::shuffle(v.begin(), v.end(), m);
  std::copy(v.begin(), v.end(), perm);
  return ELEMDP_OK;
}
const char* elemdp_kernel_name(void) { return "k4_out"; }

}
```

### rnaelem_amd/csrc/kernels.h

```cpp
#pragma once
#include <hip/hip_runtime_api.h>

#include <cstddef>
#include <cstdint>

#include "device_layout.h"
#include "energy_tables.h"
#include "bpp_cand.h"
#include "live_blocks.h"

namespace elemdp {

constexpr int kThreads = 256;

struct PlanArrays {
  int16_t* dmin = nullptr;
  double* e_stack = nullptr; double* e_ext = nullptr; double* e_ml = nullptr; double* e_close = nullptr; double* e_hp = nullptr;
  int32_t* by_outer_off = nullptr; int32_t* by_inner_off = nullptr; int32_t* by_left_off = nullptr; int32_t* by_right_off = nullptr;
  int32_t* cursor = nullptr;
  LoopItem* items = nullptr;
  uint8_t* item_in = nullptr;
  int32_t* by_inner_idx = nullptr; int32_t* by_left_idx = nullptr; int32_t* by_right_idx = nullptr;
  LoopItem* items_inner = nullptr; LoopItem* items_left = nullptr; LoopItem* items_right = nullptr;
  uint8_t* useful = nullptr;
// ... 145 lines not shown
  double* seq_out; int32_t out_stride;
  int32_t pass, d;
};
struct BppOut {
  uint32_t* okbits_out;
  int32_t* kept;
  double* lnbpp;
  double log_min_bpp;
};
constexpr int kBppLinMaxSpan = 200;
constexpr int kBppInPlanes = 7 + BC_CLASSES + 1, kBppOutPlanes = 5 + BC_CLASSES;
struct BppLinArgs {
  const EnergyTables* et;
  const EnergyTables* xet;
  const BppCandTable* cand;
  int16_t* plist; int32_t* poff;
  int32_t poff_stride, pmax;
  int32_t lmax, wmax;
  unsigned long long* prof;
  const SeqPlan* plans;
  const uint8_t* seq;
  const uint32_t* okbits;
  int16_t* dmin;
  double* xw; size_t xw_stride;
  double* tin; double* tout; size_t t_stride;
  double* lo_in; double* lo_out;
  int32_t no_ene, min_span, m_min, d;
  uint32_t* okbits_out;
  int32_t* kept;
  double* lnbpp;
  double log_min_bpp;
};
hipError_t launch_bpp_lin(const BppLinArgs& a, int G, int Lmax, int Wmax, hipStream_t st);
struct LinArgs {
  AutomatonLayout lay;
  const AutomatonLayout* layp;
  const int32_t* ints;
  const double* params;
  const double* lin;
  int32_t no_prf, m_min, no_rss;
  const SeqPlan* plans;
  const int32_t* grp;
  const SeqPlan* plans_slot;
  BatchArrays b;
  const double* ews;
  const uint32_t* okbits;
  PlanArrays p;
  const double* xwc; size_t xwc_stride;
  const double* xwi; size_t xwi_stride;
  double* band_in; double* band_out; double* ext_in; double* ext_out;
  size_t band_stride, ext_stride;
  double* zs;
  double* seq_out; int32_t out_stride;
  int32_t schedule, pass, d;
  int32_t cpb;
  float rcp_nap, rcp_lane, rcp_cpb;
  int32_t* flagged;
  int32_t lik_ratio;
  int32_t scan;
  int32_t* ys; int32_t* ye;
  double* pos_start; double* pos_inner; double* pos_end; double* exist;
  TraceRec* tr_ext; int32_t* sc_psihat; char* sc_rss; int32_t* trace_stack; int32_t trace_stack_stride;
  long long* prof;
  double* a_in; double* a_out; size_t a_stride;
  const uint32_t* okbits_end;
  int32_t lmax, nword_max;
  int32_t wmax;
  int32_t n_stage;
  int32_t dbg;
  int32_t ext_ring;
  int32_t ext_block;
  int32_t n_lin;
  int32_t fast;
  int32_t det;
  int32_t cyk_compact;
  int32_t det_sh;
  double* det_rows; int32_t det_nslot;
  int32_t live_span;
  const int32_t* blk_grid;
  int32_t loop_pre = 0, in_d0 = 0;
  const int32_t* blk_grid_in = nullptr;
  int32_t loop_post = 0;
  int32_t scan_terms = 0, range_all = 0;
};
struct LinWeightArgs {
  const LoopItem* items_inner; const LoopItem* items_left; const LoopItem* items_right;
  const double* e_stack; const double* e_ext; const double* e_ml; const double* e_close; const double* e_hp;
  const LoopItem* items;
  size_t n_cells, n_items;
  size_t cell_first = 0, cell_count = 0;
  const double* params;
  double* xwc; double* xwi;
};
hipError_t launch_lin_weights(const LinWeightArgs& a, hipStream_t st);
enum ScanPass { SCAN_PASS_START = 0, SCAN_PASS_END = 1, SCAN_PASS_INSIDE = 2, SCAN_PASS_OUT_ARI = 3, SCAN_PASS_OUT_NASI = 4 };
hipError_t launch_lin_scan_group(const LinArgs& full, int G, int Lmax, int Wmax, ScanPass pass, hipStream_t st);
hipError_t launch_cyk_group(const LinArgs& full, int G, int Lmax, int Wmax, hipStream_t st);
hipError_t launch_lin_group(const LinArgs& full, int G, int Lmax, int Wmax, bool first_pass_only, hipStream_t st);
hipError_t launch_bpp_group(const TrArgs& base, const BppOut& o, int G, int Lmax, int Wmax, hipStream_t st);
hipError_t launch_train_group(const TrArgs& base, int G, int Lmax, int Wmax, hipStream_t st);

hipError_t launch_mask(const BatchArrays& b, const SeqPlan* plans, int n_seq, int min_span, bool write_bits, uint32_t* okbits,
                       int32_t* n_canonical, hipStream_t st);
hipError_t launch_plan_cells(const PlanKernelArgs& a, int32_t* n_items_out, hipStream_t st);
hipError_t launch_plan_items(const PlanKernelArgs& a, hipStream_t st);
hipError_t launch_useful_mask(const PlanKernelArgs& a, size_t n_cells, size_t lds_cap, hipStream_t st);
void useful_mask_host(const uint8_t* kept, const uint8_t* unp, int L, int W, int C, int m_min, bool no_ene, uint8_t* out);
hipError_t launch_live_blocks(const PlanKernelArgs& a, size_t n_records, hipStream_t st);
void live_blocks_host(const uint8_t* mask, int L, int W, int cpb, int cap, int32_t* counts, LiveBlock* records, int stride, int bits = 0xff);
bool lin_loop_prepass_ok(const AutomatonLayout& lay, const int32_t* ints, int min_span);
bool lin_loop_outside_ok(const AutomatonLayout& lay, const int32_t* ints);
int lin_train_cpb(const LinArgs& full);
int lin_live_span_max();
hipError_t launch_plan_sort(const PlanKernelArgs& a, hipStream_t st);
hipError_t launch_permute_items(const PlanKernelArgs& a, hipStream_t st);
bool plan_copies_fused(const PlanKernelArgs& a);
hipError_t launch_dp(int kind, const DpArgs& a, int n_blocks, hipStream_t st);
hipError_t launch_reduce(const double* seq_out, int out_stride, int n_seq, int n_theta, double* partial, hipStream_t st);
const char* dp_kernel_name(int kind);

struct PairArgs {
  const SeqPlan* plans;
  const int32_t* idx;
  const uint32_t* okbits;
  const double* band_in; const double* band_out; size_t band_stride;
  int32_t p_cs, p_rs, ncol;
  const double* zs;
  const double* seq_out; int32_t out_stride;
  int32_t skip_flagged;
  double* P; size_t p_stride;
  double min_prob;
  double* unpaired;
  const int64_t* koff;
  int32_t* st_i; int32_t* st_j; double* st_p;
  int64_t* cnt;
  double mea_gamma2;
  double* mea_M; int32_t* mea_ch; size_t mea_ch_stride;
  char* mea_s; double* mea_score;
};
hipError_t launch_pair_cells(const PairArgs& a, int G, int cells_max, hipStream_t st);
hipError_t launch_pair_seq(const PairArgs& a, int G, hipStream_t st);
hipError_t launch_pair_mea(const PairArgs& a, int G, int Wmax, hipStream_t st);

struct CondArgs {
  const SeqPlan* plans;
  const int32_t* idx;
  const uint32_t* okbits;
  const double* band_in; const double* band_out; size_t band_stride;
  int32_t p_cs, p_rs, ncol;
  const double* z; int32_t z_log;
  const double* seq_out; int32_t out_stride;
  int32_t skip_flagged;
  double* P[2]; size_t p_stride;
  double min_prob;
  double* unpaired[2];
  double* exist; double* shift;
  const int64_t* koff;
  int32_t* st_i; int32_t* st_j; double* st_p[2];
  int64_t* cnt;
};
hipError_t launch_cond_cells(const CondArgs& a, int world, int G, int cells_max, hipStream_t st);
hipError_t launch_cond_seq(const CondArgs& a, int G, hipStream_t st);
hipError_t launch_cond_scatter(const int64_t* koff, const int64_t* cnt, const int64_t* off, const int32_t* st_i, const int32_t* st_j,
                               const double* st_p0, const double* st_p1, int n, int32_t* seq, int32_t* i, int32_t* j, double* p0,
                               double* p1, hipStream_t st);

// ... 14 lines not shown
```

### rnaelem_amd/csrc/lin_kernels.hip

```cpp
#include <hip/hip_runtime.h>

#include <algorithm>
#include <cstdio>
#include <cstdlib>
#include <type_traits>

#ifndef ELEMDP_KCI
#define ELEMDP_KCI 2
#endif
#ifndef ELEMDP_LB_IN
#define ELEMDP_LB_IN 4
#endif
#ifndef ELEMDP_LB_IN_FAST
#define ELEMDP_LB_IN_FAST 8
#endif
#ifndef ELEMDP_LB_CYK
#define ELEMDP_LB_CYK 8
#endif
#ifndef ELEMDP_LB_OUT6
#define ELEMDP_LB_OUT6 6
#endif
#ifndef ELEMDP_LB_OUT
#define ELEMDP_LB_OUT 4
#endif
// ... 418 lines not shown
  int hi = nc - 1;
  while (lo < hi) {
    const int mid = (lo + hi + 1) >> 1;
    if (pre[mid] <= p) lo = mid; else hi = mid - 1;
  }
  n = base[lo] + (p - pre[lo]);
}
struct RecAhead { LoopItem it; int meta; bool have; };
__device__ __forceinline__ RecAhead outer_fetch_ahead(const LViews& v, int n_rec, int nc, int tid, const int* pre, const int* base) {
  RecAhead r;
  r.have = tid < n_rec;
  r.meta = 0;
  r.it = LoopItem{0., 0, 0, 0, 0};
  if (r.have) {
    int lo, n;
    outer_locate(tid, nc, pre, base, lo, n);
    const bool in = v.q.item_in[n] != 0;
    r.it = v.q.items[n];
    r.meta = (in ? 0 : (int)0x80000000) | (lo << 16) | (tid - pre[lo]);
  }
  return r;
}
template <bool WEIGHTS, bool AHEAD = false>
__device__ __forceinline__ void outer_stage(const LViews& v, const OuterRecs& r, int p0, int np, int nc, int tid, const int* pre,
                                            const int* base, const RecAhead ahead = RecAhead{LoopItem{0., 0, 0, 0, 0}, 0, false}) {
  for (int x = tid; x < np; x += kBT) {
    const int p = p0 + x;
    LoopItem itv;
    int meta;
    if (AHEAD && p == tid && ahead.have) { itv = ahead.it; meta = ahead.meta; }
    else {
      int lo, n;
      outer_locate(p, nc, pre, base, lo, n);
      const bool in = v.q.item_in[n] != 0;
      itv = v.q.items[n];
      meta = (in ? 0 : (int)0x80000000) | (lo << 16) | (p - pre[lo]);
    }
    r.it[x] = itv;
    if (WEIGHTS) {
      const double tsc = itv.tsc;
      r.xw[x] = meta >= 0 ? lin_weight(v.m.lambda[0], tsc) : 0.;
      r.xw[r.cap + x] = meta >= 0 ? lin_weight(v.m.lambda[1], tsc) : 0.;
    }
    r.meta[x] = meta;
  }
  __syncthreads();
}

__device__ __forceinline__ bool block_is_dead(const SeqView& q, int d, int i0, int nc, int tid, int bits = UB_ALL) {
  if (!q.useful) return false;
  const int b = tid < nc ? ((int)q.useful[d * (q.L + 1) + i0 + tid] & bits) : 0;
  return !__syncthreads_or(b);
}
__device__ __forceinline__ void fill_dead_rows(const TableView& T, int d, int i0, int nc, int tid, int e0, int e1, int e2, int e3) {
  const int pl[4] = {e0, e1, e2, e3};
#pragma unroll
  for (int k = 0; k < 4; ++k) {
    if (pl[k] < 0) continue;
    double* row = T.band + T.cidx(pl[k], d, i0, 0);
    for (int t = tid; t < nc * T.rs[pl[k]]; t += kBT) row[t] = 0.;
  }
  if (T.ap) {
    double* row = T.ap + T.aidx(d, i0, 0);
    for (int t = tid; t < nc * T.nAs; t += kBT) row[t] = 0.;
  }
}

__device__ __forceinline__ void fill_dead_cells(const TableView& T, unsigned long long live, int first, int d, int lo, int hi, int tid,
                                                int e0, int e1, int e2, int e3) {
  auto dead = [&](int i) { const int k = i - first; return k < 0 || k > 63 || !((live >> k) & 1ull); };
  auto plane = [&](int e) {
    if (e < 0) return;
    const int rs = T.rs[e];
    double* row = T.band + T.cidx(e, d, lo, 0);
    for (int t = tid; t < (hi - lo) * rs; t += kBT) if (dead(lo + t / rs)) row[t] = 0.;
  };
  plane(e0); plane(e1); plane(e2); plane(e3);
  if (T.ap) {
    double* row = T.ap + T.aidx(d, lo, 0);
    for (int t = tid; t < (hi - lo) * T.nAs; t += kBT) if (dead(lo + t / T.nAs)) row[t] = 0.;
  }
}
struct LiveCells { int i0, nc, span, own_lo, own_end; unsigned long long live; bool sweep; };
__device__ __forceinline__ LiveCells live_cells(const SeqView& q, int d, int bx, int ncell) {
  LiveCells r;
  const int nslot = live_blocks_slots(q.L), slot = bx < nslot ? bx : nslot - 1;
#if defined(__HIP_DEVICE_COMPILE__)
  typedef const LiveBlock __attribute__((address_space(4))) * ConstBlock;
  const LiveBlock b = *reinterpret_cast<ConstBlock>(reinterpret_cast<uintptr_t>(q.blocks + live_blocks_at(q.L, q.W, d) + slot));
#else
  const LiveBlock b = q.blocks[live_blocks_at(q.L, q.W, d) + slot];
#endif
  r.sweep = slot == bx && b.count > 0;
  r.i0 = r.sweep ? b.first : 0;
  r.nc = r.sweep ? b.count : 0;
  r.live = r.sweep ? b.live : 0ull;
  r.span = r.sweep ? 64 - __builtin_clzll(b.live | 1ull) : 0;
  r.own_lo = r.sweep ? b.own_lo : 0;
  r.own_end = r.sweep ? b.own_end : (bx == 0 ? ncell : 0);
  return r;
}

template <bool BIG, bool CON, bool FAST = false, int FP = kFastP, bool W8 = false, bool LISTS = false, bool LPRE = false>
__global__ __launch_bounds__(kBT, W8 ? ELEMDP_LB_IN_FAST : ELEMDP_LB_IN) void k4_in(LinArgs a) {
  extern __shared__ double lds[];
  PhaseClock pc;
  pc.start(a.prof);

  unsigned bx, by;
  swizzled_block(bx, by);
  LViews v(a.lay);
  make_lviews(a, by, v);
  const AutomatonLayout& A = a.lay;
  const int S = a.lay.S, NA = a.lay.n_active, d = a.d, cpb = a.cpb, tid = threadIdx.x;
  if (d > v.q.W) return;
  constexpr bool MASK = FAST && !CON;
  const int ncell = v.q.L - d + 1;
  static_assert(!LISTS || (FAST && !CON), "lists: the table-driven train form only");
  static_assert(!LPRE || (FAST && !CON), "loop pre-pass: the table-driven train form only");
  constexpr int kDeadL = LPRE ? -1 : (int)ST_L;
  constexpr bool lists = LISTS;
  int i0 = bx * cpb, nc = 0, span = 0;
  unsigned long long live = 0ull;
  if (lists) {
    const LiveCells lc = live_cells(v.q, d, (int)bx, ncell);
    if (lc.own_end - lc.own_lo > lc.nc) fill_dead_cells(v.in, lc.live, lc.i0, d, lc.own_lo, lc.own_end, tid, kDeadL, ST_2, ST_1, ST_M);
    if (!lc.sweep) return;
    i0 = lc.i0; nc = lc.nc; span = lc.span; live = lc.live;
  } else {
    if (i0 >= ncell) return;
    nc = span = (cpb < ncell - i0) ? cpb : ncell - i0;
  }
  if (CON) {
    const int ys = a.ys[v.n];
    if (ys < i0 || ys - d + 1 > i0 + nc - 1) return;
  }
  if (MASK && !lists && block_is_dead(v.q, d, i0, nc, tid, LPRE ? (UB_ALL & ~UB_L) : UB_ALL)) { fill_dead_rows(v.in, d, i0, nc, tid, kDeadL, ST_2, ST_1, ST_M); return; }
  const int HD = FAST ? A.n_lane : S;
  const int CS = cpb * HD;
  constexpr int NW = 1;
  double* hb = lds;
  double* he = hb + CS;
  double* hbA = hb;
  double* heA = he;
  double* st1 = lds + NW * 2 * CS;
  const int SP = (MASK && a.live_span > cpb) ? a.live_span : cpb;
  const BlockLds BL = block_lds(NW * 2 * CS + kRecIn, cpb, a.n_lin, SP + a.wmax + 3, FAST ? a.lay.fb_in_n : staged_ints(a.lay, a.n_stage, 0), 0, FAST ? kCellInD : 0, SP);
  int* lof = reinterpret_cast<int*>(reinterpret_cast<unsigned char*>(lds) + BL.lof);
  const bool gaps = lists && (live & (live + 1ull)) != 0ull;
  if (gaps) {
    if (tid < 64 && ((live >> tid) & 1ull)) lof[__popcll(live & ((1ull << tid) - 1ull))] = tid;
    __syncthreads();
  }
  auto ci = [&](int c) -> int { return (LISTS && gaps) ? i0 + lof[c] : i0 + c; };
  constexpr int kCRin = (ELEMDP_CPB_MAX * 8 + kBT - 1) / kBT;
  double crx[kCRin];
  if (FAST) {
#pragma unroll
    for (int r = 0; r < kCRin; ++r) {
      crx[r] = 0.;
      if (r * kBT < cpb * 8) {
        const int t = tid + r * kBT, c = (t >> 3) < nc ? (t >> 3) : 0;
        crx[r] = cell_in_fetch(v.q, d, ci(c), t & 7);
      }
    }
  }
  if (a.dbg & 1024) { if (nc == 12345) lds[tid] = crx[0]; return; }
  const BlockCtx cx = stage_context<BIG, 0, FAST>(a, v, reinterpret_cast<unsigned char*>(lds), BL, i0, span, d, cpb, gaps ? ci(tid < nc ? tid : 0) : -1);
  int* dm = cx.dm; int* cnts = cx.cnts; int* pre = cx.pre; int* base = cx.base;
  const int32_t* G = v.m.big;
  double* crec = reinterpret_cast<double*>(reinterpret_cast<unsigned char*>(lds) + BL.crec);
  int* crfl = reinterpret_cast<int*>(reinterpret_cast<unsigned char*>(lds) + BL.crfl);
  for (int t = tid; t < NW * 2 * CS; t += kBT) lds[t] = 0.;
  __syncthreads();
  if (a.dbg & 2048) return;
  pc.mark<0>();
  if (FAST) {
#pragma unroll
    for (int r = 0; r < kCRin; ++r) {
      const int t = tid + r * kBT, c = t >> 3, k = t & 7;
      if (c < nc) {
        const bool on = k < 4 ? v.q.pair_ok(ci(c), d) : v.q.e_ok(ci(c), d);
        crec[c * kCellInD + 2 + k] = on ? crx[r] : 0.;
      }
    }
    for (int c = tid; c < nc; c += kBT) {
      const int i = ci(c), j = i + d;
      int fl = cell_in_flags(v.m, v.q, d, i);
      if (CON) { const int ys = a.ys[v.n]; fl |= (i == ys ? CF_YL : 0) | (j - 1 == ys ? CF_YR : 0); }
      crfl[c] = fl;
      crec[c * kCellInD] = v.q.ews[i];
      crec[c * kCellInD + 1] = v.q.ews[j > 0 ? j - 1 : 0];
    }
  }
  const double* B = v.in.band;
  const int nq = ((a.dbg & 2) || (ELEMDP_KO & 2)) ? 0 : A.n_quad;
  outer_ranges_load(v, i0, nc, d, nq > 0, tid, cnts, base, gaps ? lof : nullptr);
  const RecAhead ahead{LoopItem{0., 0, 0, 0, 0}, 0, false};
  {
    const int nA = A.n_ap;
    const int32_t* I = v.m.ints;
    const Constraint con{CON ? a.ys[v.n] : -1, -1, 0};
    const int W1 = v.q.W + 1;
    const int pad = (a.det && a.det_sh >= 0) ? (1 << a.det_sh) : nA;
    const int nwork = ((a.dbg & 1) || (ELEMDP_KO & 1)) ? 0 : nc * pad;
    const bool one_wave = a.det && a.det_sh < 0;
    for (int w = one_wave ? ((tid < 64) ? tid : nwork) : tid; w < nwork; w += one_wave ? 64 : kBT) {
      const int c = (a.det && a.det_sh >= 0) ? (w >> a.det_sh) : div_rcp(w, a.rcp_nap), p = w - c * pad;
      if (p >= nA) continue;
      const int i = ci(c), j = i + d;
      if (FAST) {
        const int32_t* PR = G + A.fpr_in + 8 * p;
        const int r0 = PR[0], r1 = PR[1];
        const int c1 = fcol(r0, 0), cP = fcol(r0, 1), tg = (r0 >> 16) & 0xff;
        const int dmi = dm[c];
        double av = 0.;
        const bool exists = dmi > 0 && dmi < d;
        const bool dead = MASK && exists && !(v.q.ubits(i, d) & UB_A);
        if (dead) {
          v.in.a(d, i, p) = 0.;
        } else if (exists) {
          BitIter it;
          it.init(v.q.okbits_end, j * W1, 1, d - dmi);
          const int nch = (dmi < d - 1 && v.q.unp[j - 1]) ? (r1 >> 16) & 15 : 0;
          int ce[kFastR];
          double pv[kFastR];
#pragma unroll
          for (int u = 0; u < kFastR; ++u) {
            ce[u] = PR[2 + u];
            pv[u] = v.in.lda(d - 1, i, u < nch ? ce[u] & 0xff : p, u < nch);
          }
          bool first = true;
          for (;;) {
            int sp[kStems];
            sp[0] = it.next();
            if (sp[0] < 0 && !first) break;
#pragma unroll
            for (int u = 1; u < kStems; ++u) sp[u] = sp[u - 1] < 0 ? -1 : it.next();
            double sa[kStems], sb[kStems];
#pragma unroll
            for (int u = 0; u < kStems; ++u) {
              const bool g = sp[u] >= 0;
              const int q = g ? sp[u] : 1;
              sa[u] = v.in.ldc(ST_1, d - q, i, c1, g);
              sb[u] = v.in.ldc(ST_B, q, j - q, cP, g);
            }
            if (first) {
              first = false;
              const double wt = (r0 & (2 << 24)) ? v.q.ews[j - 1] : 1.;
              const int bj = v.q.seq[j - 1];
#pragma unroll
              for (int u = 0; u < kFastR; ++u)
                if (u < nch) {
                  const int id = (ce[u] >> 8) & 0x7fff;
                  if (CON && j - 1 == con.ys && !(G[A.fs_in + id] & SF_SR)) continue;
                  av = fma(pv[u], v.m.lin[A.lin_wr + 5 * id + bj] * wt, av);
                }
            }
#pragma unroll
            for (int u = 0; u < kStems; ++u) av = fma(sa[u], sb[u], av);
            if (sp[kStems - 1] < 0) break;
          }
          v.in.a(d, i, p) = av;
        }
        if (tg != 0xff && av != 0.) atomicAdd(&hbA[c * HD + tg], av);
        continue;
      }
      const int s1 = I[A.ap_s1 + p], t = I[A.ap_t + p], tgt = I[A.ap_tgt + p];
      const int c1 = v.in.col(ST_1, s1), cP = v.in.col(ST_P, t);
      const int dmi = dm[c];
      double av = 0.;
      if (dmi > 0 && dmi < d) {
        const double* xml = v.q.xwc + (size_t)(lamk(v.m, t) * 5 + XT_ML) * v.q.xwc_stride;
        BitIter it;
        it.init(v.q.okbits_end, j * W1, 1, d - dmi);
        const int e0 = I[A.ap_chain_off + p], ne = v.q.unp[j - 1] ? I[A.ap_chain_off + p + 1] - e0 : 0;
        double pv[kUnary];
        const bool tail = dmi < d - 1;
#pragma unroll
        for (int u = 0; u < kUnary; ++u) pv[u] = v.in.lda(d - 1, i, u < ne ? I[A.ap_chain_ent + 2 * (e0 + u)] : p, tail);
        bool first = true;
        for (;;) {
          const int sp0 = it.next();
          if (sp0 < 0) {
            if (!first) break;
          }
          if (first) {
            first = false;
#pragma unroll
            for (int u = 0; u < kUnary; ++u)
              if (u < ne) {
                const int pc2 = I[A.ap_chain_ent + 2 * (e0 + u)], tf = I[A.ap_chain_ent + 2 * (e0 + u) + 1];
                if (!CON || allow_right(v.m, con, v.q.L, j, t, I[A.ap_t + pc2])) av = fma(pv[u], lw_right(v.m, v.q, t, tf, j - 1), av);
              }
            for (int u = kUnary; u < ne; ++u) {
              const int pc2 = I[A.ap_chain_ent + 2 * (e0 + u)], tf = I[A.ap_chain_ent + 2 * (e0 + u) + 1];
              if (CON && !allow_right(v.m, con, v.q.L, j, t, I[A.ap_t + pc2])) continue;
              av = fma(v.in.lda(d - 1, i, pc2, tail), lw_right(v.m, v.q, t, tf, j - 1), av);
            }
            if (sp0 < 0) break;
          }
          const int sp1 = it.next(), sp2 = (sp1 < 0) ? -1 : it.next(), sp3 = (sp2 < 0) ? -1 : it.next();
          const int q1 = sp1 < 0 ? sp0 : sp1, q2 = sp2 < 0 ? sp0 : sp2, q3 = sp3 < 0 ? sp0 : sp3;
// ... 470 lines not shown
  }
  __syncthreads();
  if (KB > 1) {
    for (int i0 = v.q.L - 1; i0 >= 0; i0 -= KB) {
      const int ia = i0 - blk;
      if (part < nparts && ia >= 0) s_part[tid] = lin_outside_ext_pairs<MODE>(x, ia, ps, part, nparts);
      __syncthreads();
      for (int b = 0; b < KB && i0 - b >= 0; ++b) {
        const int i = i0 - b;
        if (tid < S) {
          double t = lin_outside_ext_rule8<MODE>(x, i, tid);
          for (int k = 0; k < nparts; ++k) t += s_part[b * 128 + k * S + tid];
          v.out.o(i, tid) = t;
          if (n_ring > 0) Or.o(i, tid) = t;
        }
        __syncthreads();
      }
    }
  } else
  for (int i = v.q.L - 1; i >= 0; --i) {
    if (S <= 128) {
      if (part < nparts) s_part[tid] = lin_outside_ext_part<MODE>(x, i, ps, part, nparts);
      __syncthreads();
      if (tid < S) {
        double t = 0.;
        for (int k = 0; k < nparts; ++k) t += s_part[k * S + tid];
        v.out.o(i, tid) = t;
        if (n_ring > 0) Or.o(i, tid) = t;
      }
    } else {
      for (int s = tid; s < S; s += 128) lin_outside_ext_target<MODE>(x, i, s);
    }
    __syncthreads();
  }
  if (MODE == OUT_TRAIN || MODE == OUT_SCAN) lflush(a, v, pi, sink, l_stat, NT, a.det_nslot - 1);
}

__global__ __launch_bounds__(kThreads) void k4_r7(LinArgs a) {
  __shared__ AutomatonLayout s_lay;
  stage_layout(a, &s_lay, kThreads);
  LViews v(s_lay);
  make_lviews(a, blockIdx.y, v);
  __syncthreads();
  const AutomatonLayout& A = s_lay;
  const int L = v.q.L, W = v.q.W, S = A.S;
  const int c = blockIdx.x * kThreads + threadIdx.x;
  if (c >= (L + 1) * (W + 1)) return;
  const int i = c / (W + 1), d = c - i * (W + 1);
  if (!v.q.pair_ok(i, d)) return;
  const int j = i + d;
  const int32_t* G = v.m.big;
  const double x0 = xw_cell(v.q, 0, XT_EXT, v.q.cell(i, d)), x1 = xw_cell(v.q, 1, XT_EXT, v.q.cell(i, d));
  for (int s = 0; s < S; ++s) {
    double acc = 0.;
    for (int u = G[A.split2_off + s]; u < G[A.split2_off + s + 1]; ++u) {
      const int par = G[A.split2_ent + 2 * u], s2i = G[A.split2_ent + 2 * u + 1];
      acc = fma(v.out.o(j, par), v.in.o(i, s2i) * (lamk(v.m, par) ? x1 : x0), acc);
    }
    v.out.st(ST_P, d, i, s, acc);
  }
}

template <int MODE, bool BIG, bool FAST = false, int FP = kFastP, bool W6 = false, bool LISTS = false, bool LPOST = false>
__global__ __launch_bounds__(kBT, W6 ? ELEMDP_LB_OUT6 : ELEMDP_LB_OUT) void k4_out(LinArgs a) {
  extern __shared__ double lds[];
  PhaseClock pc;
  pc.start(a.prof);

  unsigned bx, by;
  swizzled_block(bx, by);
  LViews v(a.lay);
  make_lviews(a, by, v);
  const LPass pi = lpass(a, v);
  const AutomatonLayout& A = a.lay;
  const int S = a.lay.S, NA = a.lay.n_active, d = a.d, cpb = a.cpb, tid = threadIdx.x, nt = a.lay.n_theta;
  if (d > v.q.W) return;
  const int L = v.q.L, W = v.q.W;
  constexpr bool MASK = FAST && MODE == OUT_TRAIN;
  const int ncell = L - d + 1;
  static_assert(!LISTS || (FAST && MODE == OUT_TRAIN), "lists: the table-driven train form only");
  static_assert(!LPOST || (FAST && MODE == OUT_TRAIN), "the L plane behind the sweep: the table-driven train form only");
  constexpr int kDeadL = LPOST ? -1 : ST_L;
  constexpr bool lists = LISTS;
  int i0 = bx * cpb, nc = 0, span = 0;
  unsigned long long live = 0ull;
  if (lists) {
    const LiveCells lc = live_cells(v.q, d, (int)bx, ncell);
    if (lc.own_end - lc.own_lo > lc.nc) fill_dead_cells(v.out, lc.live, lc.i0, d, lc.own_lo, lc.own_end, tid, kDeadL, ST_2, ST_M, -1);
    if (!lc.sweep) return;
    i0 = lc.i0; nc = lc.nc; span = lc.span; live = lc.live;
  } else {
    if (i0 >= ncell) return;
    nc = span = (cpb < ncell - i0) ? cpb : ncell - i0;
  }
  if (MODE == OUT_END) {
    if (!(a.dbg & 4096) && i0 + nc - 1 + d <= a.ys[v.n]) return;
  }
  if (MASK && !lists && block_is_dead(v.q, d, i0, nc, tid, LPOST ? (UB_ALL & ~UB_L) : UB_ALL)) { fill_dead_rows(v.out, d, i0, nc, tid, kDeadL, ST_2, ST_M, -1); return; }
  const int HD = FAST ? A.n_lane : S;
  const int CS = cpb * HD;
  constexpr int NW = 1;
  const int NWS = a.det ? kBT / 64 : 1, wvd = a.det ? tid >> 6 : 0;
  const int HS = 4 * CS, ES = 2 * nt + 4;
  double* h1 = lds;
  double* h2 = h1 + CS;
  double* hp = h2 + CS;
  double* hl = hp + CS;
  double* h1A = h1;
  double* h2A = h2;
  double* hpA = hp;
  double* l_en0 = lds + HS;
  double* l_en = l_en0 + wvd * ES;
  double* l_eh = l_en + 2 * nt;
  double* l_pos = l_en0 + NWS * ES;
  const int SP = (MASK && a.live_span > cpb) ? a.live_span : cpb;
  const int win = SP + a.wmax + 3;
  constexpr bool kScanMode = MODE == OUT_SCAN || MODE == OUT_END;
  double* sOB1 = l_pos + (kScanMode ? 2 * win : 0);
  const BlockLds BL = block_lds(out_doubles(CS, nt, win, NWS, kScanMode), cpb, a.n_lin, win, FAST ? a.lay.fb_out_n : staged_ints(a.lay, a.n_stage, 1), 3 * cpb, FAST ? kCellOutD : 0, SP);
  int* lof = reinterpret_cast<int*>(reinterpret_cast<unsigned char*>(lds) + BL.lof);
  const bool gaps = lists && (live & (live + 1ull)) != 0ull;
  if (gaps) {
    if (tid < 64 && ((live >> tid) & 1ull)) lof[__popcll(live & ((1ull << tid) - 1ull))] = tid;
    __syncthreads();
  }
  auto ci = [&](int c) -> int { return (LISTS && gaps) ? i0 + lof[c] : i0 + c; };
  constexpr int kCRout = (ELEMDP_CPB_MAX * 12 + kBT - 1) / kBT;
  double crx[kCRout];
  if (FAST) {
#pragma unroll
    for (int r = 0; r < kCRout; ++r) {
      crx[r] = 0.;
      if (r * kBT < cpb * 12) {
        const int t = tid + r * kBT, c0 = t / 12, c = c0 < nc ? c0 : 0;
        crx[r] = cell_out_fetch(v.q, d, ci(c), t - c0 * 12);
      }
    }
  }
  if (a.dbg & 1024) { if (nc == 12345) lds[tid] = crx[0] + pi.invZ; return; }
  const BlockCtx cx = stage_context<BIG, 1, FAST>(a, v, reinterpret_cast<unsigned char*>(lds), BL, i0, span, d, cpb, gaps ? ci(tid < nc ? tid : 0) : -1);
  if (pi.skip) return;
  int* dm = cx.dm; int* cnts = cx.cnts; int* pre = cx.pre; int* base = cx.base;
  const int32_t* G = v.m.big;
  double* crec = reinterpret_cast<double*>(reinterpret_cast<unsigned char*>(lds) + BL.crec);
  int* crfl = reinterpret_cast<int*>(reinterpret_cast<unsigned char*>(lds) + BL.crfl);
  const int n_zero = HS + NWS * ES + ((MODE == OUT_SCAN || MODE == OUT_END) ? 2 * win : 0);
  for (int t = tid; t < n_zero; t += kBT) lds[t] = 0.;
  __syncthreads();
  if (a.dbg & 2048) return;
  pc.mark<5>();
  if (FAST) {
#pragma unroll
    for (int r = 0; r < kCRout; ++r) {
      const int t = tid + r * kBT, c = t / 12, k = t - c * 12;
      if (c < nc) {
        const int i = ci(c);
        const bool on = k < 4 ? v.q.e_ok(i, d) : k < 6 ? v.q.pair_ok(i, d) : k < 8 ? (v.q.pair_ok(i - 1, d + 2) && v.q.pair_ok(i, d)) : true;
        crec[c * kCellOutD + 2 + k] = on ? crx[r] : 0.;
      }
    }
    for (int c = tid; c < nc; c += kBT) {
      const int i = ci(c), j = i + d;
      int fl = cell_out_flags(v.m, v.q, d, i);
      if (MODE == OUT_END) { const int ys = a.ys[v.n]; fl |= (i - 1 == ys ? CF_YL : 0) | (j == ys ? CF_YR : 0) | (L == j + 1 ? CF_JLAST : 0); }
      crfl[c] = fl;
      crec[c * kCellOutD] = v.q.ews[i > 0 ? i - 1 : 0];
      crec[c * kCellOutD + 1] = v.q.ews[j < L ? j : L];
    }
  }
  LinSink sink;
  sink.en_ = l_en;
  sink.eh0 = sink.eh1 = 0.;
  const int pos_p0 = (i0 > 0) ? i0 - 1 : 0;
  if (MODE == OUT_SCAN) { sink.pos0 = l_pos - pos_p0; sink.pos1 = l_pos + win - pos_p0; }
  if (MODE == OUT_END) sink.pos2 = l_pos - pos_p0;
  const TableView& in = v.in;
  const TableView& out = v.out;
  const int nq = ((a.dbg & 2) || (ELEMDP_KO & 2)) ? 0 : A.n_quad;
  const double* IB = in.band;
  const double* OB = out.band;
  for (int vc = tid; vc < 3 * cpb; vc += kBT) {
// ... 186 lines not shown
          double x0[kTU], x1[kTU], x2[kTU], aux[kTU];
#pragma unroll
          for (int u = 0; u < kTU; ++u) {
            const bool on = k0 + u < n_mine;
            const int kk = on ? k0 + u : 0;
            const int t = !on ? (nq > wv ? wv : 0) : a.det ? G[qd0 + 5 + m0 + kk] : wv + kWaves * kk;
            qa[u] = G[qc0 + 2 * t];
            qb[u] = on ? G[qc0 + 2 * t + 1] : (4 << 16);
            x0[u] = OB[rE + (qa[u] & 0xff)]; x1[u] = IB[r1 + ((qa[u] >> 8) & 0xff)]; x2[u] = IB[r2 + ((qa[u] >> 16) & 0xff)];
            aux[u] = role == 0 ? IB[rA + ((qa[u] >> 24) & 0xff)] : 1.;
          }
#pragma unroll
          for (int u = 0; u < kTU; ++u) {
            const double term = x0[u] * (x1[u] * x2[u]) * ((qb[u] & (1 << 16)) ? xw1 : xw0);
            if ((qb[u] & (4 << 16)) || !valid || aux[u] == 0. || term == 0.) continue;
            atomicAdd(&hrow[qb[u] & 0xffff], term);
            if (MODE == OUT_TRAIN && role == 0) {
              const bool w1 = pi.merged && (qb[u] & (2 << 16));
              const bool k1 = !v.m.lam_same && (qb[u] & (1 << 16));
              const double w = it.tsc * term * (aux[u] * (w1 ? pi.invZs : pi.invZ));
              ew[0] += (!w1 && !k1) ? w : 0.;
              ew[1] += (!w1 && k1) ? w : 0.;
              ew[2] += (w1 && !k1) ? w : 0.;
              ew[3] += (w1 && k1) ? w : 0.;
            }
          }
        }
      }
      __syncthreads();
      pc.mark<9>();
    }
    if (MODE == OUT_TRAIN && n_rec > 0) {
#pragma unroll
      for (int k = 0; k < 4; ++k) {
        const double e = wave_sum(ew[k]);
        if ((tid & 63) == 0 && e != 0.) atomicAdd(&l_eh[k], e);
      }
    }
  }
  pc.mark<10>();
  const int NL = FAST ? A.n_lane : NA;
  const int end_ys = (MODE == OUT_END && !(a.dbg & 4096)) ? a.ys[v.n] : -1;
  if (tid < nc * NL && !(a.dbg & 4) && !(ELEMDP_KO & 4)) {
    const int c = div_rcp(tid, a.rcp_lane);
    const int s = FAST ? G[A.f_live_out + tid - c * NL] : tid - c * NL;
    const int slot = FAST ? tid : c * HD + s;
    double oB = 0.;
    if (ci(c) + d > end_ys) {
      const bool w1 = pi.merged && s == A.shadow;
      sink.world = w1 ? 1 : 0;
      sink.en_ = l_en + (w1 ? nt : 0);
      if (FAST) {
        oB = fast_outside_unary<kFastR, FP, kFastL, MODE, LPOST>(A, G + A.fp_out + s * kFastW, G, v.m.lin, in, out, crec + c * kCellOutD, crfl[c],
                                                          d, ci(c), w1 ? pi.invZs : pi.invZ, v.m.lam_same != 0, v.m.no_prf != 0, sink,
                                                          h1 + slot, CS, NW, HS, G + A.fs_out);
      } else {
        LinOutCtx<LinSink> x{v.m, v.q, in, out, w1 ? pi.invZs : pi.invZ, sink, Constraint{MODE == OUT_END ? a.ys[v.n] : -1, -1, 0}};
        HeavyOut H;
        H.H1 = rep_sum(h1 + slot, NW, HS); H.H2 = rep_sum(h2 + slot, NW, HS);
        H.HP = rep_sum(hp + slot, NW, HS); H.HL = rep_sum(hl + slot, NW, HS);
        if (!(a.dbg & 32)) H.HP += out.ld(ST_P, d, i0 + c, s, v.q.pair_ok(i0 + c, d));
        H.ext_in_hp = true;
        oB = lin_outside_target_u<MODE>(x, d, i0 + c, s, H);
      }
    }
    hp[slot] = oB;
  }
  __syncthreads();
  if (!(a.dbg & 1) && !(a.dbg & 128) && !(ELEMDP_KO & 8)) {
    const int nA = A.n_ap;
    double* const en_keep = sink.en_;
    for (int w = tid; w < nc * nA; w += kBT) {
      const int c = div_rcp(w, a.rcp_nap), p = w - c * nA;
      if (ci(c) + d <= end_ys) continue;
      if (FAST) {
        const int32_t* PR = G + A.fpr_out + 8 * p;
        const int r0 = PR[0], r1 = PR[1];
        const int tg = (r0 >> 16) & 0xff;
        const bool w1 = pi.merged && (r0 & (4 << 24));
        const int i = ci(c), j = i + d, dmi = dm[c];
        const bool exists = dmi > 0 && dmi < d;
        const bool dead = MASK && exists && !((crfl[c] >> CF_USH) & UB_A);
        if (dead) {
          out.a(d, i, p) = 0.;
        } else if (exists) {
          const bool step = d + 1 <= W && j < L && v.q.unp[j];
          const int nr = step ? (r1 >> 20) & 15 : 0;
          const double a_in = in.a(d, i, p);
          int ce[kFastR];
          double op[kFastR];
#pragma unroll
          for (int u = 0; u < kFastR; ++u) {
            ce[u] = PR[5 + u];
            op[u] = out.lda(d + 1, i, u < nr ? ce[u] & 0xff : p, u < nr);
          }
          double acc = 0.;
          if (a_in != 0.) {
            acc = tg != 0xff ? hp[c * HD + tg] : 0.;
            const double inz = a_in * (w1 ? pi.invZs : pi.invZ);
            const int bj = step ? (int)v.q.seq[j] : 0;
            const double ewj = step ? v.q.ews[j] : 1.;
            double* en = l_en + (w1 ? nt : 0);
#pragma unroll
            for (int u = 0; u < kFastR; ++u)
              if (u < nr) {
                const int id = (ce[u] >> 8) & 0x7fff;
                const double term = op[u] * (v.m.lin[A.lin_wr + 5 * id + bj] * ((G[A.fe_r + 2 * id + 1] & 1) ? ewj : 1.));
                const double z = term * inz;
                if ((MODE == OUT_SCAN || MODE == OUT_END) &&
                    !fast_scan_stat<MODE, false, true>(sink, G[A.fs_out + id], i - 1, j, false, MODE == OUT_END && j == a.ys[v.n], L == j + 1, z))
                  continue;
                if (MODE != OUT_END && !v.m.no_prf && z != 0. && bj) atomicAdd(&en[G[A.fe_r + 2 * id] + bj], z);
                acc += term;
              }
          }
          out.a(d, i, p) = acc;
        }
        continue;
      }
      const int tgt = v.m.ints[A.ap_tgt + p];
      const bool w1 = pi.merged && v.m.ints[A.ap_t + p] == A.shadow;
      sink.en_ = l_en + (w1 ? nt : 0);
      LinOutCtx<LinSink> x{v.m, v.q, in, out, w1 ? pi.invZs : pi.invZ, sink, Constraint{MODE == OUT_END ? a.ys[v.n] : -1, -1, 0}};
      lin_outside_apair<MODE>(x, d, i0 + c, p, tgt >= 0 ? hp[c * HD + tgt] : 0.);
    }
    sink.en_ = en_keep;
  }
  pc.mark<11>();
  if (MODE == OUT_SCAN || MODE == OUT_END) {
    __syncthreads();
    const int p1 = (i0 + nc + d < L) ? i0 + nc + d : L;
    for (int t = tid; t <= p1 - pos_p0; t += kBT) {
      const double v0 = l_pos[t], v1 = l_pos[win + t];
      if (MODE == OUT_SCAN) {
        if (v0 != 0. && pos_p0 + t < L) atomicAdd(&a.pos_start[v.seq_base + pos_p0 + t], v0);
        if (v1 != 0. && pos_p0 + t < L) atomicAdd(&a.pos_inner[v.seq_base + pos_p0 + t], v1);
      } else if (v0 != 0.) {
        atomicAdd(&a.pos_end[v.pos_base + pos_p0 + t], v0);
      }
    }
  }
  if (MODE == OUT_TRAIN || MODE == OUT_SCAN) lflush(a, v, pi, sink, l_en0, kBT, (int)bx);
  pc.mark<12>();
  pc.finish();
}

constexpr int kRowsT = 8, kRowsMax = 32, kSeedCap = 256, kSeedBatch = 2;
static_assert(2 * kRowsMax <= 64, "the runs of a tile are scanned by one wave");
__host__ __device__ inline int loop_rows_r(int rs) { const int r = kBT / (rs > 0 ? rs : 1); return r < kRowsMax ? r : kRowsMax; }
static size_t loop_rows_lds(const AutomatonLayout& A) {
  const size_t rs = A.tab_rs[ST_L], R = loop_rows_r(A.tab_rs[ST_L]);
  return sizeof(double) * (R * (kRowsT + 1) * rs + 2 * kSeedCap + (R + kRowsT) + 5 * (size_t)A.n_wr + 2 * (size_t)A.n_theta + 4) +
         sizeof(int32_t) * (2 * R * (kRowsT + 1) + 2 * R + 1 + 4 * kSeedCap + 4 * (size_t)A.n_quad + (size_t)A.n_lane + kLoopColsMax * (kLoopProgW + 1) + (R + kRowsT));
}
__global__ __launch_bounds__(kBT) void k4_out_lrows(LinArgs a) {
  extern __shared__ double lds[];
  unsigned bx, by;
  swizzled_block(bx, by);
  LViews v(a.lay);
  make_lviews(a, by, v);
  const LPass pi = lpass(a, v);
  if (pi.skip) return;
  const AutomatonLayout& A = a.lay;
  const int tid = threadIdx.x, L = v.q.L, W = v.q.W, nt = A.n_theta, nq = A.n_quad, HD = A.n_lane;
  const int rs = v.out.rs[ST_L], R = loop_rows_r(rs), TS = (kRowsT + 1) * rs;
  const int i0 = bx * R;
  if (i0 > L) return;
// ... 621 lines not shown
bool lin_loop_prepass_ok(const AutomatonLayout& A, const int32_t* ints, int min_span) {
  const bool say = getenv("ELEMDP_PLAN_DEBUG") != nullptr;
  if (!A.fp_ok || A.tab_rs[ST_L] < 1 || A.tab_rs[ST_L] > kLoopColsMax || loop_prepass_lds(A) > 64 * 1024) {
    if (say) fprintf(stderr, "loop pre-pass: not for this automaton (fp_ok %d, L row of %d columns)\n", A.fp_ok, A.tab_rs[ST_L]);
    return false;
  }
  auto col = [](int packed, int byte) { const int c = (packed >> (8 * byte)) & 0xff; return c == 0xff ? -1 : c; };
  unsigned seen = 0;
  for (int k = 0; k < A.n_lane; ++k) {
    const int32_t* P = ints + A.fp_in + ints[A.f_live_in + k] * kFastW;
    const int c = col(P[2], 2);
    if (c >= 0) {
      if (c >= A.tab_rs[ST_L] || ((seen >> c) & 1u)) { if (say) fprintf(stderr, "loop pre-pass: not for this automaton (column %d of lane %d)\n", c, k); return false; }
      seen |= 1u << c;
      continue;
    }
    if (!(P[0] & 1) || col(P[1], 1) < 0) continue;
    const int nR = (P[0] >> 8) & 15;
    bool zero = !(P[0] & 2) || min_span > 2;
    for (int u = 0; u < nR && u < kFastR; ++u) zero = zero && col(P[4 + u], 0) < 0;
    if (!zero) { if (say) fprintf(stderr, "loop pre-pass: not for this automaton (lane %d: a loop state with an E column, no L column and an L value)\n", k); return false; }
  }
  return true;
}
static bool loop_outside_lds_ok(const AutomatonLayout& A) {
  return A.tab_rs[ST_L] >= 1 && A.tab_rs[ST_L] <= kLoopColsMax && A.tab_rs[ST_L] <= kBT && loop_rows_lds(A) <= 64 * 1024;
}
bool lin_loop_outside_ok(const AutomatonLayout& A, const int32_t* ints) {
  const bool say = getenv("ELEMDP_PLAN_DEBUG") != nullptr;
  if (!A.fp_ok || !loop_outside_lds_ok(A)) {
    if (say) fprintf(stderr, "L kernel behind the outside sweep: not for this automaton (fp_ok %d, L row of %d columns, LDS %zu)\n", A.fp_ok, A.tab_rs[ST_L], loop_rows_lds(A));
    return false;
  }
  auto col = [](int packed, int byte) { const int c = (packed >> (8 * byte)) & 0xff; return c == 0xff ? -1 : c; };
  unsigned seen = 0;
  for (int k = 0; k < A.n_lane; ++k) {
    const int s = ints[A.f_live_out + k];
    const int c = col(ints[A.fp_out + s * kFastW + 2], 2), ci = col(ints[A.fp_in + s * kFastW + 2], 2);
    if (c != ci || (c >= 0 && (c >= A.tab_rs[ST_L] || ((seen >> c) & 1u)))) {
      if (say) fprintf(stderr, "L kernels behind the outside sweep: not for this automaton (state %d: L column %d outside, %d inside)\n", s, c, ci);
      return false;
    }
    if (c >= 0) seen |= 1u << c;
  }
  return true;
}
static GroupGeom group_geometry(const LinArgs& full, int G, int Lmax, int Wmax, bool scan) {
  GroupGeom g;
  LinArgs& a = g.a;
  a = full;
  const int S = a.lay.S, nt = a.lay.n_theta;
  a.cpb = std::min(kBT / S, ELEMDP_CPB_MAX);
  a.wmax = Wmax;
  a.ext_ring = G <= 1024 ? 1 : 0;
  a.lmax = Lmax;
  if (scan) { a.schedule = 0; a.pass = 0; a.scan = 1; a.det = 0; }
  g.big = a.n_stage >= a.lay.n_ints;
  const bool fast = g.fast = geometry_fast(a);
  a.fast = fast ? 1 : 0;
  if (fast) a.cpb = std::min(kBT / std::max(a.lay.n_lane, 1), ELEMDP_CPB_MAX);
  a.n_lin = fast ? a.lay.lin_total : kLinEth + nt;
  const int NW = a.det ? kBT / 64 : 1;
  g.hd = fast ? a.lay.n_lane : S;
  set_rcps(a, fast);
  if (scan || !fast || a.det || !a.p.useful || !a.p.blocks || !a.blk_grid || a.live_span < a.cpb) { a.p.blocks = nullptr; a.blk_grid = nullptr; a.live_span = 0; }
  if (scan || !fast || !a.p.useful) a.loop_pre = 0;
  if (a.loop_pre && a.p.blocks && (!a.p.blocks_in || !a.blk_grid_in)) a.loop_pre = 0;
  if (scan || !fast || !a.p.useful || a.det) a.loop_post = 0;
  if (a.loop_post && a.p.blocks && (!a.p.blocks_in || !a.blk_grid_in)) a.loop_post = 0;
  if (a.loop_post && !loop_outside_lds_ok(a.lay)) a.loop_post = 0;
  const int sp = a.live_span > a.cpb ? a.live_span : a.cpb;
  g.win = sp + Wmax + 3;
  g.lds_in = block_lds(2 * a.cpb * g.hd + kRecIn, a.cpb, a.n_lin, g.win, fast ? a.lay.fb_in_n : staged_ints(a.lay, a.n_stage, 0), 0, fast ? kCellInD : 0, sp).total;
  g.lds_out = block_lds(out_doubles(a.cpb * g.hd, nt, g.win, NW, scan), a.cpb, a.n_lin, g.win, fast ? a.lay.fb_out_n : staged_ints(a.lay, a.n_stage, 1), 3 * a.cpb, fast ? kCellOutD : 0, sp).total;
  g.stage_ext = Lmax <= 2048 && a.nword_max <= 8192;
  g.lds_ext_in = g.stage_ext ? (size_t)ext_lds((a.ext_ring ? ext_ring_doubles(0, Wmax, S, kLinEth + nt, Lmax, a.nword_max, a.n_stage) : 0), kLinEth + nt, Lmax, a.nword_max, a.n_stage).total : 0;
  g.ext_nt = (a.ext_block == kExtBlock && a.ext_ring && a.lay.n_active <= 128 && !(a.dbg & 8192)) ? 128 * kExtBlock : 128;
  return g;
}
static unsigned band_blocks(LinArgs& a, int ncell, bool train) {
  const int n = (ncell + a.cpb - 1) / a.cpb;
  if (!train || !a.blk_grid || !a.p.blocks) return (unsigned)n;
  if (a.blk_grid[a.d] < 0) { a.p.blocks = nullptr; return (unsigned)n; }
  return (unsigned)std::max(1, std::min(n, a.blk_grid[a.d]));
}
template <bool CON>
static void inside_sweeps(GroupGeom& g, int G, int Lmax, int Wmax, bool bands, hipStream_t st) {
  LinArgs& a = g.a;
  const bool pre = !CON && bands && g.fast && a.loop_pre;
  LinArgs ai = a;
  if (!pre) ai.loop_pre = 0;
  if (pre) {
    if (a.p.blocks) { ai.p.blocks = a.p.blocks_in; ai.blk_grid = a.blk_grid_in; }
    hipLaunchKernelGGL(k4_in_loops, dim3((Lmax + kLoopLanes) / kLoopLanes, G), dim3(kLoopLanes), loop_prepass_lds(a.lay), st, ai);
  }
  if (bands)
    for (int d = pre ? a.in_d0 : 0; d <= Wmax; ++d) {
      const int ncell = Lmax - d + 1;
      if (ncell <= 0) break;
      LinArgs ad = ai;
      ad.d = d;
      const unsigned gx = band_blocks(ad, ncell, !CON);
      launch_k4_in<CON>(ad, dim3(gx, G), g.lds_in, g.fast, g.big, st);
    }
  if (g.stage_ext) hipLaunchKernelGGL((k4_in_ext<true, CON>), dim3(G), dim3(g.ext_nt), g.lds_ext_in, st, a);
  else hipLaunchKernelGGL((k4_in_ext<false, CON>), dim3(G), dim3(128), 0, st, a);
}
template <int MODE>
static void outside_bands(GroupGeom& g, int G, int Lmax, int Wmax, hipStream_t st) {
  LinArgs& a = g.a;
  hipLaunchKernelGGL(k4_r7, dim3(((Lmax + 1) * (Wmax + 1) + kThreads - 1) / kThreads, G), dim3(kThreads), 0, st, a);
  const bool post = MODE == OUT_TRAIN && g.fast && a.loop_post;
  LinArgs ao = a;
  if (!post) ao.loop_post = 0;
  if (post && a.p.blocks) { ao.p.blocks = a.p.blocks_in; ao.blk_grid = a.blk_grid_in; }
  for (int d = Wmax; d >= (post ? a.in_d0 : 0); --d) {
    const int ncell = Lmax - d + 1;
    if (ncell <= 0) continue;
    LinArgs ad = ao;
    ad.d = d;
    const unsigned gx = band_blocks(ad, ncell, MODE == OUT_TRAIN);
    launch_k4_out<MODE>(ad, dim3(gx, G), g.lds_out, g.fast, g.big, st);
  }
  if (post) {
    const int rows = loop_rows_r(a.lay.tab_rs[ST_L]);
    hipLaunchKernelGGL(k4_out_lrows, dim3((Lmax + rows) / rows, G), dim3(kBT), loop_rows_lds(a.lay), st, a);
  }
}
template <int MODE>
static void scan_outside(GroupGeom& g, int G, int Lmax, int Wmax, hipStream_t st) {
  const LinArgs& a = g.a;
  const int S = a.lay.S, nt = a.lay.n_theta;
  const size_t lds_ext_out = g.stage_ext ? (size_t)ext_lds(2 * nt + 4 + (a.ext_ring ? ext_ring_doubles(2 * nt + 4, Wmax, S, kLinEth + nt, Lmax, a.nword_max, a.n_stage) : 0), kLinEth + nt, Lmax, a.nword_max, a.n_stage).total : sizeof(double) * (2 * nt + 4);
  if (g.stage_ext) hipLaunchKernelGGL((k4_out_ext<MODE, true>), dim3(G), dim3(g.ext_nt), lds_ext_out, st, a);
  else hipLaunchKernelGGL((k4_out_ext<MODE, false>), dim3(G), dim3(128), lds_ext_out, st, a);
  outside_bands<MODE>(g, G, Lmax, Wmax, st);
}
template <bool CON, int MODE>
static void scan_sweeps(GroupGeom& g, int G, int Lmax, int Wmax, hipStream_t st) {
  inside_sweeps<CON>(g, G, Lmax, Wmax, true, st);
  scan_outside<MODE>(g, G, Lmax, Wmax, st);
}

hipError_t launch_lin_scan_group(const LinArgs& full, int G, int Lmax, int Wmax, ScanPass pass, hipStream_t st) {
  if (G <= 0) return hipSuccess;
  GroupGeom g = group_geometry(full, G, Lmax, Wmax, true);
  const LinArgs& a = g.a;
  if (getenv("ELEMDP_LDS_DEBUG") && pass == SCAN_PASS_START) fprintf(stderr, "scan group: G %d cpb %d S %d nt %d fast %d n_lin %d fast blob in/out %d/%d ints win %d lds k4_in %zu k4_out %zu\n", G, a.cpb, a.lay.S, a.lay.n_theta, (int)g.fast, a.n_lin, a.lay.fb_in_n, a.lay.fb_out_n, g.win, g.lds_in, g.lds_out);
  if (pass == SCAN_PASS_INSIDE) {
    inside_sweeps<false>(g, G, Lmax, Wmax, true, st);
  } else if (pass == SCAN_PASS_START) {
    scan_sweeps<false, OUT_SCAN>(g, G, Lmax, Wmax, st);
    hipLaunchKernelGGL(k5_pick<0>, dim3((G + 63) / 64), dim3(64), 0, st, a, G);
  } else if (pass == SCAN_PASS_OUT_ARI || pass == SCAN_PASS_OUT_NASI) {
    g.a.scan_terms = pass == SCAN_PASS_OUT_ARI ? 1 : 2;
    scan_outside<OUT_SCAN>(g, G, Lmax, Wmax, st);
  } else {
    scan_sweeps<true, OUT_END>(g, G, Lmax, Wmax, st);
    hipLaunchKernelGGL(k5_pick<1>, dim3((G + 63) / 64), dim3(64), 0, st, a, G);
  }
  return hipGetLastError();
}

hipError_t launch_lin_group(const LinArgs& full, int G, int Lmax, int Wmax, bool first_pass_only, hipStream_t st) {
  if (G <= 0) return hipSuccess;
  GroupGeom g = group_geometry(full, G, Lmax, Wmax, false);
  const LinArgs& a = g.a;
  const int S = a.lay.S, nt = a.lay.n_theta;
  inside_sweeps<false>(g, G, Lmax, Wmax, !a.no_rss, st);
  const int n_pass = (a.schedule == 1 || first_pass_only) ? 1 : 2;
  const bool combine = (a.schedule == 1 || a.lik_ratio || a.det) && !first_pass_only;
  if (getenv("ELEMDP_LDS_DEBUG")) {
    const bool stats = !(g.big && (a.dbg & 16));
    fprintf(stderr, "lin group: G %d cpb %d fast %d n_lin %d staged ints in/out %d/%d lds k4_in %zu k4_out %zu fp_max_p %d forms k4_in %s k4_out %s stage_ext %d ext_nt %d ext_ring %d n_pass %d combine %d\n", G, a.cpb, (int)g.fast, a.n_lin, staged_ints(a.lay, a.n_stage, 0), staged_ints(a.lay, a.n_stage, 1), g.lds_in, g.lds_out, a.lay.fp_max_p,
            a.no_rss ? "none" : kK4FormName[k4_form(a, g.lds_in, 8, g.fast, g.big)], a.no_rss ? "none" : !stats ? "nostat" : kK4FormName[k4_form(a, g.lds_out, 6, g.fast, g.big)],
            (int)g.stage_ext, g.stage_ext ? g.ext_nt : 128, a.ext_ring, n_pass, (int)combine);
    fprintf(stderr, "lin group: loop_prepass %d loop_outside %d (k4_out_lrows lds %zu, %d rows x %d diagonals)\n", a.loop_pre, a.loop_post, loop_rows_lds(a.lay), loop_rows_r(a.lay.tab_rs[ST_L]), kRowsT);
  }
  for (int pass = 0; pass < n_pass; ++pass) {
    GroupGeom gp = g;
    LinArgs& b = gp.a;
    b.pass = pass;
    const int n_stat = ext_stat_doubles(nt, b.det);
    if (g.stage_ext) hipLaunchKernelGGL((k4_out_ext<OUT_TRAIN, true>), dim3(G), dim3(b.det ? 128 : g.ext_nt), (size_t)ext_lds(n_stat + (b.ext_ring ? ext_ring_doubles(n_stat, Wmax, S, kLinEth + nt, Lmax, b.nword_max, b.n_stage) : 0), kLinEth + nt, Lmax, b.nword_max, b.n_stage).total, st, b);
    else hipLaunchKernelGGL((k4_out_ext<OUT_TRAIN, false>), dim3(G), dim3(128), sizeof(double) * n_stat, st, b);
    if (b.no_rss) continue;
    if (g.big && (b.dbg & 16)) outside_bands<OUT_NONE>(gp, G, Lmax, Wmax, st);
    else outside_bands<OUT_TRAIN>(gp, G, Lmax, Wmax, st);
  }
  if (combine) hipLaunchKernelGGL(k4_combine, dim3(G), dim3(kThreads), 0, st, a, G);
  return hipGetLastError();
}

}
```

### rnaelem_amd/csrc/slot_sizing.h

```cpp
#pragma once
#include <algorithm>
#include <cstddef>

#include "device_layout.h"

namespace elemdp {

struct SlotRequest {
  int S = 0;
  int row = 0;
  bool scan = false;
  int n_want = 0;
  int group = 0;
  int opt_slots = 0, n_cu = 0;
  int pair_row = 0;
  int Lmax = 0, Wmax = 0;
  int S_dense = 0;
  size_t budget = 0;

  size_t cells() const { return (size_t)(Wmax + 1) * (Lmax + 1); }
  size_t band() const { return cells() * (row > 0 ? row : kNumBandStates * S); }
  size_t ext() const { return (size_t)(Lmax + 1) * S; }
  size_t dense1() const { return (size_t)kNumBandStates * (Wmax + 1) * (Lmax + 1) * S_dense; }
  size_t per_slot() const {
    return (band() + ext()) * 2 * sizeof(double) + (scan ? ext() * sizeof(TraceRec) + 16 * (size_t)(Lmax + 2) : 0);
  }
  int want() const { return std::max(1, std::min(group > 0 ? group : opt_slots > 0 ? opt_slots : 2 * n_cu, n_want)); }
};

struct SlotGeometry {
  int n = 0, S = 0;
  bool trace = false;
  size_t band_stride = 0;
};

inline int trace_stack_stride(int Lmax) { return 4 * (4 * (Lmax + 2)); }

inline bool slots_keep(const SlotGeometry& g, const SlotRequest& r) {
  return g.n >= r.want() && g.S == r.S && g.band_stride == r.band() && (g.trace || !r.scan);
}

inline int slots_sized(const SlotRequest& r, size_t free_b, size_t held_b) {
  const size_t per_slot = r.per_slot();
  int want = r.want();
  size_t budget = (size_t)((double)(free_b + held_b) * 0.72);
  if (r.budget > 0) budget = std::min(budget, r.budget);
  if (per_slot * (size_t)want > budget) want = (int)std::max<size_t>(1, budget / per_slot);
  if (per_slot * want > free_b + held_b) return 0;
  return want;
}

inline int even_groups(int n, long n_slots) {
  const long n_groups = (n + n_slots - 1) / n_slots;
  return (int)((n + n_groups - 1) / n_groups);
}

inline int balanced_group(size_t per_slot_bytes, int n, int group_cap, int opt_group, size_t budget_in, size_t free_b, size_t held_b) {
  if (opt_group > 0) return opt_group;
  size_t budget = (size_t)((double)(free_b + held_b) * 0.68);
  if (budget_in > 0) budget = std::min(budget, budget_in);
  long cap = (long)(budget / std::max<size_t>(per_slot_bytes, 1));
  cap = std::max(1L, std::min(cap, (long)group_cap));
  return even_groups(n, cap);
}

inline size_t lin_group_bytes(int Lmax, int Wmax, int row, int Sa, int nap) {
  const size_t cells = (size_t)(Wmax + 1) * (Lmax + 1), ext = (size_t)(Lmax + 1);
  return (cells * row + ext * Sa) * 2 * sizeof(double) + ext * Sa * 3 * sizeof(double) + cells * nap * 2 * sizeof(double);
}

}
```

### rnaelem_amd/csrc/table_slots.h

```cpp
#pragma once
#include "device_buf.h"
#include "slot_sizing.h"

namespace elemdp {

struct TableSlots {
  enum class Holds { Nothing, DenseLog, Linear, Trace };
  enum class Held { Group, Slots, Stream };

  DevBuf band_in, band_out, ext_in, ext_out, tmp;
  DevBuf tr_ext, tr_stack;
  DevBuf zs, a_in, a_out;

  int n() const { return holds_ == Holds::Trace ? 0 : g_.n; }
  size_t band_stride() const { return g_.band_stride; }
  Holds holds() const { return holds_; }
  int linear_S() const { return linear_S_; }
  void set_holds(Holds h, int linear_S = 0) { holds_ = h; linear_S_ = linear_S; }

  size_t held_bytes(Held set) const {
    const size_t band = band_in.bytes() + band_out.bytes(), ext = ext_in.bytes() + ext_out.bytes();
    switch (set) {
      case Held::Group: return band + ext;
      case Held::Slots: return band + ext + tmp.bytes() + tr_ext.bytes() + tr_stack.bytes();
      default: return band;
    }
  }

  void ensure(const SlotRequest& r, size_t free_b) {
    if (holds_ == Holds::Trace) invalidate();
    Lmax_ = r.Lmax; S_dense_ = r.S_dense;
    if (!slots_keep(g_, r)) {
      const int n = slots_sized(r, free_b, held_bytes(Held::Slots));
      if (n < 1) throw HipError("not enough device memory for one table slot");
      invalidate();
      const size_t band = std::max(r.band() * n, r.dense1()) * sizeof(double);
      band_in.alloc(band);
      band_out.alloc(band);
      ext_in.alloc(r.ext() * n * sizeof(double));
      ext_out.alloc(r.ext() * n * sizeof(double));
      tmp.alloc(r.ext() * 3 * n * sizeof(double));
      g_.n = n; g_.S = r.S; g_.band_stride = r.band();
      if (r.scan) { ensure_trace(); g_.trace = true; }
    }
    if (r.pair_row > 0) {
      zs.alloc(sizeof(double) * 4 * g_.n);
      a_in.alloc(sizeof(double) * r.cells() * r.pair_row * g_.n);
      a_out.alloc(sizeof(double) * r.cells() * r.pair_row * g_.n);
    }
  }
  void ensure_trace() {
    tr_ext.alloc((size_t)(Lmax_ + 1) * S_dense_ * g_.n * sizeof(TraceRec));
    tr_stack.alloc((size_t)g_.n * trace_stack_stride(Lmax_) * sizeof(int32_t));
  }
  void invalidate() { g_ = SlotGeometry(); set_holds(Holds::Nothing); }
  void release() {
    for (DevBuf* d : {&band_in, &band_out, &ext_in, &ext_out, &tmp, &tr_ext, &tr_stack, &zs, &a_in, &a_out}) d->reset();
    invalidate();
  }

 private:
  SlotGeometry g_;
  Holds holds_ = Holds::Nothing;
  int linear_S_ = 0, Lmax_ = 0, S_dense_ = 0;
};

}
```

Before: 50710 seq/s.

## Keep dead-cell zeros resident across train evals with per-sequence owned slots

Each sequence gets its own table slot when memory allows, so the band tables persist between training evaluations. A binding records the plan, slot generation and options, and when the next eval matches it the kernels skip rewriting dead cells to zero and skip launching diagonals that have no live blocks. This removes repeated zero-fill stores and empty launches on every iteration. In exchange it uses more device memory for one slot per sequence, and correctness depends on the binding catching every state change that could leave stale values in the tables.

```diff
diff --git a/rnaelem_amd/api.py b/rnaelem_amd/api.py
--- a/rnaelem_amd/api.py
+++ b/rnaelem_amd/api.py
@@ -490,6 +490,11 @@
         self._lib.elemdp_last_timing(self._h, _dp(ms), 3)
         return ms
 
+    def slot_status(self):
+        ms = np.zeros(5)
+        self._lib.elemdp_last_timing(self._h, _dp(ms), 5)
+        return {"zeros_kept": bool(ms[3]), "slots": int(ms[4])}
+
     def profile(self):
         c = np.zeros(16)
         self._lib.elemdp_debug_profile(self._h, _dp(c), 16)
diff --git a/rnaelem_amd/csrc/engine.cpp b/rnaelem_amd/csrc/engine.cpp
--- a/rnaelem_amd/csrc/engine.cpp
+++ b/rnaelem_amd/csrc/engine.cpp
@@ -211,6 +211,8 @@
   void debug_tables(double* inside, double* outside, double* inside_o, double* outside_o, double* ENo, double* ENx, double* EH);
   void batch_pairs(int idx, uint8_t* kept, double* lnbpp, int cap);
   double last_ms[3] = {0, 0, 0};
+  bool last_zeros_kept() const { return last_zeros_kept_; }
+  int slots_held() const { return slots_.n_held(); }
 
  private:
   void upload_params(const double* x, const AutomatonLayout& lay, bool trivial);
@@ -245,7 +247,8 @@
   void run_train();
   void run_train_batch();
   void run_lin_batch();
-  int prepare_lin(LinArgs& a, bool sched1, bool dense_too = false, int n_eval = 0, int group_cap = 8192);
+  int prepare_lin(LinArgs& a, bool sched1, bool dense_too = false, int n_eval = 0, int group_cap = 8192, bool own = false);
+  ZeroBinding zero_binding(const LinArgs& a, bool sched1, bool ranged) const;
   template <class Work> void sweep_groups(const LinArgs& a, int n, const int32_t* h_ord, const int32_t* d_ord, const SeqPlan* d_sorted,
                                           int gsz, int ns, Work work);
   struct ScanPos {
@@ -268,7 +271,7 @@
   TrArgs log_pipeline_args();
   void init_device();
   void flatten_automaton();
-  void poison_tables();
+  bool poison_tables();
   void lin_weights(int first = 0, int count = 0);
   void upload_automaton();
   bool opt_prune_ = true;
@@ -278,6 +281,11 @@
   int range_key_[2] = {-1, -1};
   bool opt_det_ = false;
   bool opt_fast_ = true;
+  bool opt_own_slots_ = true;
+  bool own_map_ = false;
+  int lock_slots_ = 0;
+  bool last_zeros_kept_ = false;
+  unsigned long long plan_gen_ = 0;
   bool opt_poison_ = false;
   void require_device() const;
   bool has_device_ = false;
@@ -576,6 +584,7 @@
   else if (key == "dbg") opt_dbg_ = (int)v;
   else if (key == "bpp_log") opt_bpp_log_ = v != 0;
   else if (key == "poison") opt_poison_ = v != 0;
+  else if (key == "own_slots") opt_own_slots_ = v != 0;
   else if (key == "fast") opt_fast_ = v != 0;
   else if (key == "deterministic") opt_det_ = v != 0;
   else if (key == "sorted_plan") opt_sorted_plan_ = v != 0;
@@ -758,6 +767,7 @@
   HIP_OK(launch_useful_mask(plan_.ka, (size_t)plan_.n_cells, (size_t)opt_useful_lds_kb_ * 1024, st_));
   plan_.useful_built = true;
   plan_.blk_cpb = plan_.blk_cap = 0;
+  ++plan_gen_;
 }
 
 bool Engine::ensure_live_blocks(int cpb, int cap, bool inside_too) {
@@ -791,6 +801,7 @@
   plan_.blk_all = opt_live_blocks_ >= 2;
   plan_.blk_two = inside_too;
   plan_.blk_cpb = cpb; plan_.blk_cap = cap;
+  ++plan_gen_;
   return true;
 }
 
@@ -800,6 +811,7 @@
   if (plan_.permuted) HIP_OK(launch_permute_items(plan_.ka, st_));
   HIP_OK(hipStreamSynchronize(st_));
   plan_.sorted = true;
+  ++plan_gen_;
 }
 
 SlotRequest Engine::slot_request(int S, int row, bool scan, int n_want, int group, int pair_row) const {
@@ -1152,6 +1164,7 @@
   d_seq_out_.alloc(sizeof(double) * (size_t)out_stride_ * n);
   HIP_OK(hipMemsetAsync(d_seq_out_.as<void>(), 0, sizeof(double) * (size_t)out_stride_ * n, st_));
   slots_.invalidate();
+  ++plan_gen_;
   HIP_OK(hipStreamSynchronize(st_));
   dbg_lap("load: weights / output buffers");
 }
@@ -1343,10 +1356,12 @@
   HIP_OK(launch_reduce(d_seq_out_.as<double>(), out_stride_, n_seq_, au_.n_theta(), d_partial_.as<double>(), st_));
 }
 
-void Engine::poison_tables() {
-  if (!opt_poison_) return;
+bool Engine::poison_tables() {
+  if (!opt_poison_) return false;
+  slots_.clear_zeros();
   for (DevBuf* b : {&slots_.band_in, &slots_.band_out, &slots_.a_in, &slots_.a_out})
     if (b->bytes()) HIP_OK(hipMemsetAsync(b->as<void>(), 0xff, b->bytes(), st_));
+  return true;
 }
 
 void Engine::lin_weights(int first, int count) {
@@ -1367,7 +1382,7 @@
   HIP_OK(launch_lin_weights(w, st_));
 }
 
-int Engine::prepare_lin(LinArgs& a, bool sched1, bool dense_too, int n_eval, int group_cap) {
+int Engine::prepare_lin(LinArgs& a, bool sched1, bool dense_too, int n_eval, int group_cap, bool own) {
   const bool shadow = sched1 && lays_.shadow >= 0;
   const AutomatonLayout& L = shadow ? lays_ : lay_;
   const int S = L.S, Sa = std::max(lay_.S, lays_.S), nap = std::max(lay_.ap_rs, lays_.ap_rs);
@@ -1376,8 +1391,15 @@
   const size_t free_b = free_device_bytes();
   const int group = balanced_group(lin_group_bytes(Lmax_, Wmax_, row, Sa, nap), n_need, group_cap, opt_group_, slot_budget_, free_b,
                                    slots_.held_bytes(TableSlots::Held::Group));
-  slots_.ensure(slot_request(Sa, row, false, n_need, group, nap), free_b);
-  const int gsz = even_groups(n_need, slots_.n());
+  SlotRequest rq = slot_request(Sa, row, false, n_need, group, nap);
+  own_map_ = own && opt_own_slots_ && !inner_ && !dense_too &&
+             own_slots_fit(n_need, lin_group_bytes(Lmax_, Wmax_, row, Sa, nap), rq.per_slot(), opt_group_, opt_slots_, slot_budget_, free_b,
+                           slots_.held_bytes(TableSlots::Held::Group), slots_.held_bytes(TableSlots::Held::Slots));
+  if (own_map_) rq.group = n_need;
+  slots_.ensure(rq, free_b);
+  if (own_map_ && slots_.n() < n_need) own_map_ = false;
+  lock_slots_ = lockstep_slots(own_map_, group, n_need, slots_.n());
+  const int gsz = even_groups(n_need, lock_slots_);
   std::memset(&a, 0, sizeof(a));
   a.lay = L;
   a.layp = shadow ? d_lays_.as<AutomatonLayout>() : d_lay_.as<AutomatonLayout>();
@@ -1425,12 +1447,10 @@
 template <class Work>
 void Engine::sweep_groups(const LinArgs& a, int n, const int32_t* h_ord, const int32_t* d_ord, const SeqPlan* d_sorted, int gsz,
                           int ns, Work work) {
-  const int slots_each = slots_.n() / ns;
-  if (ns > 1) {
-    int n_groups = (n + slots_each - 1) / slots_each;
-    n_groups = ((n_groups + ns - 1) / ns) * ns;
-    gsz = (n + n_groups - 1) / n_groups;
-  }
+  const int n_lock = own_map_ ? lock_slots_ : slots_.n();
+  const int slots_each = n_lock / ns;
+  gsz = stream_group(n, gsz, n_lock, ns);
+  if (own_map_ && slots_.n() < n) throw StateError("sweep_groups: fewer slots than sequences under the own-slot mapping");
   need_group_streams(ns);
   if (ns > 1) {
     HIP_OK(hipEventRecord(gstart_, st_));
@@ -1439,7 +1459,7 @@
   int gi = 0;
   for (int g0 = 0; g0 < n; g0 += gsz, ++gi) {
     const int k = gi % ns;
-    const size_t k0 = (size_t)k * slots_each;
+    const size_t k0 = group_slot_base(own_map_, g0, k, slots_each);
     LinArgs ak = a;
     ak.band_in += k0 * a.band_stride; ak.band_out += k0 * a.band_stride;
     ak.ext_in += k0 * a.ext_stride; ak.ext_out += k0 * a.ext_stride;
@@ -1470,13 +1490,28 @@
   return n_flagged;
 }
 
+ZeroBinding Engine::zero_binding(const LinArgs& a, bool sched1, bool ranged) const {
+  ZeroBinding z;
+  z.valid = own_map_ && !ranged && a.p.useful != nullptr && lin_train_cpb(a) > 0 && !a.no_rss && a.dbg == 0 && !opt_first_pass_only_ &&
+            !opt_profile_;
+  z.plan = plan_gen_;
+  z.slots_gen = slots_.generation(); z.n_slots = slots_.n(); z.band_stride = slots_.band_stride();
+  z.own = own_map_ ? 1 : 0; z.n_seq = n_seq_;
+  z.S = a.lay.S; z.tab_row = a.lay.tab_row; z.ap_rs = a.lay.ap_rs; z.shadow = a.lay.shadow; z.schedule = sched1 ? 1 : 0;
+  z.useful_mask = opt_useful_mask_ ? 1 : 0; z.loop_prepass = opt_loop_prepass_ ? 1 : 0; z.loop_outside = opt_loop_outside_ ? 1 : 0;
+  z.live_blocks = opt_live_blocks_; z.live_span = opt_live_span_; z.deterministic = opt_det_ ? 1 : 0; z.fast = a.fast;
+  return z;
+}
+
 void Engine::run_lin_batch() {
   const bool sched1 = opt_schedule_ == 1 && linear_ok_ && !opt_first_pass_only_ && lay_.s00 == 0 && lays_.shadow >= 0;
   LinArgs a;
   const bool ranged = opt_eval_count_ > 0 && !(opt_eval_first_ == 0 && opt_eval_count_ == n_seq_);
   const int r0 = ranged ? opt_eval_first_ : 0, n_ev = ranged ? opt_eval_count_ : n_seq_;
   if (r0 < 0 || n_ev <= 0 || r0 + n_ev > n_seq_) throw ArgError("eval_first / eval_count outside the resident batch");
-  int gsz = prepare_lin(a, sched1, false, n_ev);
+  ZeroBinding had = slots_.take_zeros();
+  last_zeros_kept_ = false;
+  int gsz = prepare_lin(a, sched1, false, n_ev, 8192, !ranged);
   if (opt_useful_mask_) ensure_useful_mask();
   a.p.useful = opt_useful_mask_ ? plan_.useful.as<uint8_t>() : nullptr;
   a.loop_pre = (opt_loop_prepass_ && opt_useful_mask_ && loop_prepass_ok(sched1)) ? 1 : 0;
@@ -1510,7 +1545,7 @@
     h_ord = h_order_r_.data();
     d_ord = d_order_r_.as<int32_t>();
     d_sorted = d_plans_sorted_r_.as<SeqPlan>();
-    gsz = even_groups(n_ev, slots_.n());
+    gsz = even_groups(n_ev, lock_slots_);
   }
   HIP_OK(hipMemsetAsync(d_seq_out_.as<double>() + (size_t)r0 * out_stride_, 0, sizeof(double) * (size_t)out_stride_ * n_ev, st_));
   HIP_OK(hipMemsetAsync(d_flagged_.as<void>(), 0, sizeof(int32_t), st_));
@@ -1524,8 +1559,10 @@
   }
   HIP_OK(hipEventRecord(ev_[1], st_));
   lin_weights(r0, n_ev);
-  poison_tables();
-  const int ns = group_streams(n_ev >= 64 && slots_.n() >= 64 && !opt_profile_);
+  if (poison_tables()) had = ZeroBinding();
+  const ZeroBinding zb = zero_binding(a, sched1, ranged);
+  a.zeros_kept = zeros_match(had, zb) ? 1 : 0;
+  const int ns = group_streams(n_ev >= 64 && lock_slots_ >= 64 && !opt_profile_);
   sweep_groups(a, n_ev, h_ord, d_ord, d_sorted, gsz, ns, [&](const LinArgs& ak, size_t, int G, int Lg, int Wg, hipStream_t st) {
     HIP_OK(launch_lin_group(ak, G, Lg, Wg, opt_first_pass_only_, st));
   });
@@ -1536,8 +1573,9 @@
     last_prof.assign(16, 0);
     for (size_t k = 0; k < hp.size(); ++k) last_prof[k % 16] += hp[k];
   }
-  if (n_flagged == 0) slots_.set_holds(TableSlots::Holds::Linear, a.lay.S);
+  if (n_flagged == 0) slots_.set_holds(TableSlots::Holds::Linear, a.lay.S, zb.valid ? &zb : nullptr);
   else slots_.set_holds(TableSlots::Holds::DenseLog);
+  last_zeros_kept_ = a.zeros_kept != 0;
   if (n_flagged > 0) {
     ensure_sorted_plan();
     TrArgs t = log_pipeline_args();
@@ -3023,6 +3061,8 @@
 int elemdp_last_timing(elemdp_handle* h, double* ms, int32_t n) {
   if (!h || !ms) return ELEMDP_EINVAL;
   for (int k = 0; k < n && k < 3; ++k) ms[k] = h->e->last_ms[k];
+  if (n > 3) ms[3] = h->e->last_zeros_kept() ? 1. : 0.;
+  if (n > 4) ms[4] = (double)h->e->slots_held();
   return ELEMDP_OK;
 }
 int elemdp_debug_profile(elemdp_handle* h, double* cycles, int32_t n) {
diff --git a/rnaelem_amd/csrc/kernels.h b/rnaelem_amd/csrc/kernels.h
--- a/rnaelem_amd/csrc/kernels.h
+++ b/rnaelem_amd/csrc/kernels.h
@@ -251,6 +251,7 @@
   const int32_t* blk_grid_in = nullptr;
   int32_t loop_post = 0;
   int32_t scan_terms = 0, range_all = 0;
+  int32_t zeros_kept = 0;
 };
 struct LinWeightArgs {
   const LoopItem* items_inner; const LoopItem* items_left; const LoopItem* items_right;
diff --git a/rnaelem_amd/csrc/lin_kernels.hip b/rnaelem_amd/csrc/lin_kernels.hip
--- a/rnaelem_amd/csrc/lin_kernels.hip
+++ b/rnaelem_amd/csrc/lin_kernels.hip
@@ -524,7 +524,7 @@
   }
 }
 struct LiveCells { int i0, nc, span, own_lo, own_end; unsigned long long live; bool sweep; };
-__device__ __forceinline__ LiveCells live_cells(const SeqView& q, int d, int bx, int ncell) {
+__device__ __forceinline__ LiveCells live_cells(const SeqView& q, int d, int bx, int ncell, bool kept) {
   LiveCells r;
   const int nslot = live_blocks_slots(q.L), slot = bx < nslot ? bx : nslot - 1;
 #if defined(__HIP_DEVICE_COMPILE__)
@@ -539,7 +539,7 @@
   r.live = r.sweep ? b.live : 0ull;
   r.span = r.sweep ? 64 - __builtin_clzll(b.live | 1ull) : 0;
   r.own_lo = r.sweep ? b.own_lo : 0;
-  r.own_end = r.sweep ? b.own_end : (bx == 0 ? ncell : 0);
+  r.own_end = r.sweep ? b.own_end : ((bx == 0 && !kept) ? ncell : 0);
   return r;
 }
 
@@ -562,11 +562,12 @@
   static_assert(!LPRE || (FAST && !CON), "loop pre-pass: the table-driven train form only");
   constexpr int kDeadL = LPRE ? -1 : (int)ST_L;
   constexpr bool lists = LISTS;
+  const bool kept = MASK && a.zeros_kept != 0;
   int i0 = bx * cpb, nc = 0, span = 0;
   unsigned long long live = 0ull;
   if (lists) {
-    const LiveCells lc = live_cells(v.q, d, (int)bx, ncell);
-    if (lc.own_end - lc.own_lo > lc.nc) fill_dead_cells(v.in, lc.live, lc.i0, d, lc.own_lo, lc.own_end, tid, kDeadL, ST_2, ST_1, ST_M);
+    const LiveCells lc = live_cells(v.q, d, (int)bx, ncell, kept);
+    if (!kept && lc.own_end - lc.own_lo > lc.nc) fill_dead_cells(v.in, lc.live, lc.i0, d, lc.own_lo, lc.own_end, tid, kDeadL, ST_2, ST_1, ST_M);
     if (!lc.sweep) return;
     i0 = lc.i0; nc = lc.nc; span = lc.span; live = lc.live;
   } else {
@@ -577,7 +578,7 @@
     const int ys = a.ys[v.n];
     if (ys < i0 || ys - d + 1 > i0 + nc - 1) return;
   }
-  if (MASK && !lists && block_is_dead(v.q, d, i0, nc, tid, LPRE ? (UB_ALL & ~UB_L) : UB_ALL)) { fill_dead_rows(v.in, d, i0, nc, tid, kDeadL, ST_2, ST_1, ST_M); return; }
+  if (MASK && !lists && block_is_dead(v.q, d, i0, nc, tid, LPRE ? (UB_ALL & ~UB_L) : UB_ALL)) { if (!kept) fill_dead_rows(v.in, d, i0, nc, tid, kDeadL, ST_2, ST_1, ST_M); return; }
   const int HD = FAST ? A.n_lane : S;
   const int CS = cpb * HD;
   constexpr int NW = 1;
@@ -660,7 +661,7 @@
         const bool exists = dmi > 0 && dmi < d;
         const bool dead = MASK && exists && !(v.q.ubits(i, d) & UB_A);
         if (dead) {
-          v.in.a(d, i, p) = 0.;
+          if (!kept) v.in.a(d, i, p) = 0.;
         } else if (exists) {
           BitIter it;
           it.init(v.q.okbits_end, j * W1, 1, d - dmi);
@@ -1297,11 +1298,12 @@
   static_assert(!LPOST || (FAST && MODE == OUT_TRAIN), "the L plane behind the sweep: the table-driven train form only");
   constexpr int kDeadL = LPOST ? -1 : ST_L;
   constexpr bool lists = LISTS;
+  const bool kept = MASK && a.zeros_kept != 0;
   int i0 = bx * cpb, nc = 0, span = 0;
   unsigned long long live = 0ull;
   if (lists) {
-    const LiveCells lc = live_cells(v.q, d, (int)bx, ncell);
-    if (lc.own_end - lc.own_lo > lc.nc) fill_dead_cells(v.out, lc.live, lc.i0, d, lc.own_lo, lc.own_end, tid, kDeadL, ST_2, ST_M, -1);
+    const LiveCells lc = live_cells(v.q, d, (int)bx, ncell, kept);
+    if (!kept && lc.own_end - lc.own_lo > lc.nc) fill_dead_cells(v.out, lc.live, lc.i0, d, lc.own_lo, lc.own_end, tid, kDeadL, ST_2, ST_M, -1);
     if (!lc.sweep) return;
     i0 = lc.i0; nc = lc.nc; span = lc.span; live = lc.live;
   } else {
@@ -1311,7 +1313,7 @@
   if (MODE == OUT_END) {
     if (!(a.dbg & 4096) && i0 + nc - 1 + d <= a.ys[v.n]) return;
   }
-  if (MASK && !lists && block_is_dead(v.q, d, i0, nc, tid, LPOST ? (UB_ALL & ~UB_L) : UB_ALL)) { fill_dead_rows(v.out, d, i0, nc, tid, kDeadL, ST_2, ST_M, -1); return; }
+  if (MASK && !lists && block_is_dead(v.q, d, i0, nc, tid, LPOST ? (UB_ALL & ~UB_L) : UB_ALL)) { if (!kept) fill_dead_rows(v.out, d, i0, nc, tid, kDeadL, ST_2, ST_M, -1); return; }
   const int HD = FAST ? A.n_lane : S;
   const int CS = cpb * HD;
   constexpr int NW = 1;
@@ -1664,7 +1666,7 @@
         const bool exists = dmi > 0 && dmi < d;
         const bool dead = MASK && exists && !((crfl[c] >> CF_USH) & UB_A);
         if (dead) {
-          out.a(d, i, p) = 0.;
+          if (!kept) out.a(d, i, p) = 0.;
         } else if (exists) {
           const bool step = d + 1 <= W && j < L && v.q.unp[j];
           const int nr = step ? (r1 >> 20) & 15 : 0;
@@ -2452,6 +2454,7 @@
   const int n = (ncell + a.cpb - 1) / a.cpb;
   if (!train || !a.blk_grid || !a.p.blocks) return (unsigned)n;
   if (a.blk_grid[a.d] < 0) { a.p.blocks = nullptr; return (unsigned)n; }
+  if (a.zeros_kept && a.blk_grid[a.d] == 0) return 0u;
   return (unsigned)std::max(1, std::min(n, a.blk_grid[a.d]));
 }
 template <bool CON>
@@ -2471,6 +2474,7 @@
       LinArgs ad = ai;
       ad.d = d;
       const unsigned gx = band_blocks(ad, ncell, !CON);
+      if (!gx) continue;
       launch_k4_in<CON>(ad, dim3(gx, G), g.lds_in, g.fast, g.big, st);
     }
   if (g.stage_ext) hipLaunchKernelGGL((k4_in_ext<true, CON>), dim3(G), dim3(g.ext_nt), g.lds_ext_in, st, a);
@@ -2490,6 +2494,7 @@
     LinArgs ad = ao;
     ad.d = d;
     const unsigned gx = band_blocks(ad, ncell, MODE == OUT_TRAIN);
+    if (!gx) continue;
     launch_k4_out<MODE>(ad, dim3(gx, G), g.lds_out, g.fast, g.big, st);
   }
   if (post) {
diff --git a/rnaelem_amd/csrc/slot_sizing.h b/rnaelem_amd/csrc/slot_sizing.h
--- a/rnaelem_amd/csrc/slot_sizing.h
+++ b/rnaelem_amd/csrc/slot_sizing.h
@@ -69,4 +69,44 @@
   return (cells * row + ext * Sa) * 2 * sizeof(double) + ext * Sa * 3 * sizeof(double) + cells * nap * 2 * sizeof(double);
 }
 
+inline int stream_group(int n, int gsz, int n_slots, int ns) {
+  if (ns <= 1) return gsz;
+  const int slots_each = std::max(1, n_slots / ns);
+  int n_groups = (n + slots_each - 1) / slots_each;
+  n_groups = ((n_groups + ns - 1) / ns) * ns;
+  return (n + n_groups - 1) / n_groups;
 }
+
+inline bool own_slots_fit(int n, size_t group_bytes, size_t per_slot_bytes, int opt_group, int opt_slots, size_t budget_in, size_t free_b,
+                          size_t held_group_b, size_t held_slots_b) {
+  if (n < 1 || (opt_group > 0 && opt_group < n) || (opt_slots > 0 && opt_slots < n)) return false;
+  auto inside = [&](size_t per, size_t reach, double frac) {
+    size_t budget = (size_t)((double)reach * frac);
+    if (budget_in > 0) budget = std::min(budget, budget_in);
+    return per * (size_t)n <= budget;
+  };
+  return inside(group_bytes, free_b + held_group_b, 0.68) && inside(per_slot_bytes, free_b + held_slots_b, 0.72);
+}
+inline int lockstep_slots(bool own, int group, int n, int n_slots) { return own ? std::max(1, std::min(group, n)) : n_slots; }
+inline size_t group_slot_base(bool own, int g0, int k, int slots_each) { return own ? (size_t)g0 : (size_t)k * slots_each; }
+
+struct ZeroBinding {
+  bool valid = false;
+  unsigned long long plan = 0;
+  unsigned slots_gen = 0;
+  int n_slots = 0;
+  size_t band_stride = 0;
+  int own = 0, n_seq = 0;
+  int S = 0, tab_row = 0, ap_rs = 0, shadow = 0, schedule = 0;
+  int useful_mask = 0, loop_prepass = 0, loop_outside = 0, live_blocks = 0, live_span = 0, deterministic = 0, fast = 0;
+};
+inline bool zeros_match(const ZeroBinding& held, const ZeroBinding& want) {
+  return held.valid && want.valid && held.plan == want.plan && held.slots_gen == want.slots_gen && held.n_slots == want.n_slots &&
+         held.band_stride == want.band_stride && held.own == want.own && held.n_seq == want.n_seq && held.S == want.S &&
+         held.tab_row == want.tab_row && held.ap_rs == want.ap_rs && held.shadow == want.shadow && held.schedule == want.schedule &&
+         held.useful_mask == want.useful_mask && held.loop_prepass == want.loop_prepass && held.loop_outside == want.loop_outside &&
+         held.live_blocks == want.live_blocks && held.live_span == want.live_span && held.deterministic == want.deterministic &&
+         held.fast == want.fast;
+}
+
+}
diff --git a/rnaelem_amd/csrc/table_slots.h b/rnaelem_amd/csrc/table_slots.h
--- a/rnaelem_amd/csrc/table_slots.h
+++ b/rnaelem_amd/csrc/table_slots.h
@@ -16,7 +16,15 @@
   size_t band_stride() const { return g_.band_stride; }
   Holds holds() const { return holds_; }
   int linear_S() const { return linear_S_; }
-  void set_holds(Holds h, int linear_S = 0) { holds_ = h; linear_S_ = linear_S; }
+  void set_holds(Holds h, int linear_S = 0, const ZeroBinding* zeros = nullptr) {
+    holds_ = h; linear_S_ = linear_S;
+    zeros_ = zeros ? *zeros : ZeroBinding();
+  }
+  const ZeroBinding& zeros() const { return zeros_; }
+  ZeroBinding take_zeros() { const ZeroBinding z = zeros_; zeros_ = ZeroBinding(); return z; }
+  void clear_zeros() { zeros_ = ZeroBinding(); }
+  unsigned generation() const { return gen_; }
+  int n_held() const { return g_.n; }
 
   size_t held_bytes(Held set) const {
     const size_t band = band_in.bytes() + band_out.bytes(), ext = ext_in.bytes() + ext_out.bytes();
@@ -28,6 +36,7 @@
   }
 
   void ensure(const SlotRequest& r, size_t free_b) {
+    clear_zeros();
     if (holds_ == Holds::Trace) invalidate();
     Lmax_ = r.Lmax; S_dense_ = r.S_dense;
     if (!slots_keep(g_, r)) {
@@ -53,7 +62,7 @@
     tr_ext.alloc((size_t)(Lmax_ + 1) * S_dense_ * g_.n * sizeof(TraceRec));
     tr_stack.alloc((size_t)g_.n * trace_stack_stride(Lmax_) * sizeof(int32_t));
   }
-  void invalidate() { g_ = SlotGeometry(); set_holds(Holds::Nothing); }
+  void invalidate() { g_ = SlotGeometry(); ++gen_; set_holds(Holds::Nothing); }
   void release() {
     for (DevBuf* d : {&band_in, &band_out, &ext_in, &ext_out, &tmp, &tr_ext, &tr_stack, &zs, &a_in, &a_out}) d->reset();
     invalidate();
@@ -62,6 +71,8 @@
  private:
   SlotGeometry g_;
   Holds holds_ = Holds::Nothing;
+  ZeroBinding zeros_;
+  unsigned gen_ = 0;
   int linear_S_ = 0, Lmax_ = 0, S_dense_ = 0;
 };
 
```

Measured after the change: 51800 seq/s (median of 6 runs). 2.2% higher.
